# TimZaman/dotaclient

Hardware: NVIDIA H100
Metric: optimizer_steps_per_sec (higher is better)
Workload: dtype f32

## Files before the change

dotaclient_b200/_lib.py:

```python
import ctypes
import os

_HERE = os.path.dirname(os.path.abspath(__file__))
LIB_PATH = os.path.join(_HERE, "libdotaclient_b200.so")

_c = ctypes
_vp, _i32, _i64, _f32, _f64, _sz = _c.c_void_p, _c.c_int, _c.c_int64, _c.c_float, _c.c_double, _c.c_size_t
_ptr5 = _c.c_void_p * 5


class GatherDesc(_c.Structure):
    _fields_ = [("src", _vp), ("dst", _vp), ("outer", _i64), ("src_cols", _i64), ("row_bytes", _i64)]

SIGNATURES = {
    "dc_version": (_i32, []),
    "dc_last_error": (_c.c_char_p, []),
    "dc_device_info": (_i32, [_c.POINTER(_i32)] * 3),
    "dc_gae_scan": (_i32, [_vp, _i32, _vp, _vp, _i32, _vp, _vp, _f64, _f64, _vp, _vp, _vp]),
    "dc_vtrace_scan": (_i32, [_vp, _i32, _vp, _vp, _vp, _vp, _i32, _vp, _vp, _f64, _f64, _f64, _f64, _vp, _vp, _vp, _vp]),
    "dc_gae_scan_indexed": (_i32, [_vp, _i32, _vp, _i64, _vp, _vp, _i32, _vp, _vp, _f64, _f64, _vp, _vp, _vp]),
    "dc_vtrace_scan_indexed": (_i32, [_vp, _i32, _vp, _i64, _vp, _vp, _vp, _vp, _i32, _vp, _vp, _f64, _f64, _f64, _f64, _vp,
                                      _vp, _vp, _vp]),
    "dc_upgo_scan": (_i32, [_vp, _i32, _vp, _vp, _vp, _vp, _i32, _vp, _vp, _f64, _f64, _f64, _vp, _vp, _vp]),
    "dc_upgo_scan_indexed": (_i32, [_vp, _i32, _vp, _i64, _vp, _vp, _vp, _vp, _i32, _vp, _vp, _f64, _f64, _f64, _vp, _vp,
                                    _vp]),
    "dc_gae_scan_heads": (_i32, [_vp, _i32, _vp, _i32, _vp, _vp, _i32, _vp, _vp, _vp, _f64, _vp, _vp, _vp]),
    "dc_gae_scan_heads_indexed": (_i32, [_vp, _i32, _vp, _i32, _vp, _i64, _vp, _vp, _i32, _vp, _vp, _vp, _f64, _vp, _vp,
                                         _vp]),
    "dc_value_heads_loss": (_i32, [_vp, _i64, _vp, _vp, _vp, _i64, _i32, _vp, _vp, _i64, _vp, _vp, _vp, _vp, _vp]),
    "dc_gather_columns": (_i32, [_c.POINTER(GatherDesc), _i32, _vp, _i64, _vp]),
    "dc_gather_columns_fill": (_i32, [_c.POINTER(GatherDesc), _i32, _vp, _i64, _vp]),
    "dc_refresh_states": (_i32, [_i32, _i32, _vp, _vp, _i64, _i64, _vp, _vp, _vp, _i64, _i64, _i64, _vp, _vp, _vp, _vp, _vp,
                                 _vp, _vp]),
    "dc_rnn_workspace_bytes": (_sz, [_i32, _i32, _i32]),
    "dc_rnn_seq_fwd": (_i32, [_i32, _vp, _vp, _vp, _vp, _vp, _i32, _i32, _i32, _vp, _vp]),
    "dc_rnn_seq_bwd": (_i32, [_i32, _vp, _vp, _vp, _vp, _vp, _vp, _vp, _vp, _vp, _i32, _i32, _i32, _vp, _vp]),
    "dc_rnn_seq_fwd_reset": (_i32, [_i32, _vp, _vp, _vp, _vp, _vp, _vp, _vp, _vp, _i32, _i32, _i32, _i32, _vp, _vp]),
    "dc_rnn_seq_bwd_reset": (_i32, [_i32, _vp, _vp, _vp, _vp, _vp, _vp, _vp, _vp, _vp, _vp, _vp, _i32, _i32, _i32, _i32, _vp,
                                    _vp]),
    "dc_gemm_tf32x3_supported": (_i32, [_i64, _i32, _i32]),
    "dc_gemm_tf32x3": (_i32, [_vp, _i32, _vp, _i32, _vp, _vp, _i32, _i64, _i32, _i32, _i32, _vp]),
    "dc_gemm_wgrad_workspace_bytes": (_sz, [_i32, _i32]),
    "dc_gemm_wgrad_tf32x3": (_i32, [_vp, _i32, _vp, _i32, _i64, _i32, _i32, _vp, _i32, _vp, _i32, _vp, _vp]),
    "dc_gemm_tf32x3_rows": (_i32, [_vp, _i32, _vp, _i32, _vp, _vp, _vp, _i32, _i64, _vp, _vp, _i32, _i32, _i32, _i32, _vp]),
    "dc_gemm_wgrad_tf32x3_rows": (_i32, [_vp, _i32, _vp, _i32, _vp, _i64, _vp, _i32, _i32, _vp, _i32, _vp, _i32, _vp, _vp]),
    "dc_unit_basic_bwd_workspace_bytes": (_sz, []),
    "dc_env_fwd": (_i32, [_vp, _vp, _vp, _vp, _i32, _i64, _vp]),
    "dc_env_bwd_workspace_bytes": (_sz, []),
    "dc_env_bwd": (_i32, [_vp, _vp, _i32, _vp, _vp, _vp, _i64, _vp, _vp]),
    "dc_unit_wgrad_routed": (_i32, [_vp, _vp, _i32, _vp, _vp, _i64, _i32, _vp, _vp, _vp, _vp]),
    "dc_unit_dgrad_fused": (_i32, [_vp, _vp, _i32, _vp, _vp, _i32, _vp, _vp, _vp, _vp, _vp, _i64, _i32, _vp, _vp, _i32, _vp, _vp]),
    "dc_unit_dgrad_fused_mask": (_i32, [_vp, _vp, _i32, _vp, _vp, _i32, _vp, _vp, _vp, _vp, _vp, _vp, _i64, _i32, _vp, _vp, _i32, _vp,
                                        _vp]),
    "dc_gemm_unit_max": (_i32, [_vp, _vp, _vp, _vp, _vp, _i32, _vp, _i64, _i32, _vp]),
    "dc_unit_embed_fwd": (_i32, [_vp, _vp, _vp, _vp, _vp, _vp, _vp, _vp, _i32, _vp, _i64, _i32, _vp]),
    "dc_unit_embed_fwd_mask": (_i32, [_vp, _vp, _vp, _vp, _vp, _vp, _vp, _vp, _vp, _i32, _vp, _i64, _i32, _vp]),
    "dc_target_unit_q_fwd": (_i32, [_vp, _i32, _c.c_void_p * 6, _vp, _vp, _vp, _i64, _vp]),
    "dc_target_unit_q_bwd": (_i32, [_vp, _c.c_void_p * 6, _vp, _vp, _vp, _i32, _i64, _vp]),
    "dc_target_unit_q_fwd_rows": (_i32, [_vp, _i32, _c.c_void_p * 6, _vp, _vp, _vp, _i64, _vp, _vp, _vp]),
    "dc_target_unit_q_bwd_rows": (_i32, [_vp, _c.c_void_p * 6, _vp, _vp, _vp, _i32, _i64, _vp, _vp, _vp]),
    "dc_target_rows_workspace_bytes": (_sz, [_i64]),
    "dc_target_rows": (_i32, [_vp, _vp, _i64, _vp, _vp, _vp, _vp, _vp]),
    "dc_rows_zero_inactive": (_i32, [_vp, _i64, _vp, _i32, _i32, _vp]),
    "dc_ppo_loss_fwd_bwd": (_i32, [_ptr5, _ptr5, _ptr5, _vp, _vp, _vp, _vp, _i64, _f32, _f32, _f32, _ptr5, _vp, _vp,
                                   _vp, _vp, _vp]),
    "dc_ppo_loss_fwd_bwd_strided": (_i32, [_ptr5, _c.c_int64 * 5, _ptr5, _ptr5, _vp, _vp, _vp, _vp, _i64, _i64, _f32, _f32, _f32,
                                           _ptr5, _c.c_int64 * 5, _vp, _i64, _vp, _vp, _vp, _vp]),
    "dc_ppo_loss_fwd_bwd_dev": (_i32, [_ptr5, _c.c_int64 * 5, _ptr5, _ptr5, _vp, _vp, _vp, _vp, _i64, _vp, _i64, _vp,
                                       _ptr5, _c.c_int64 * 5, _vp, _i64, _vp, _vp, _vp, _vp, _vp]),
    "dc_ppo_loss_fwd_bwd_masked": (_i32, [_ptr5, _c.c_int64 * 5, _ptr5, _ptr5, _vp, _vp, _vp, _vp, _i64, _vp, _vp, _i64,
                                          _vp, _ptr5, _c.c_int64 * 5, _vp, _i64, _vp, _vp, _vp, _vp, _vp]),
    "dc_ppo_loss_fwd_bwd_joint": (_i32, [_ptr5, _c.c_int64 * 5, _ptr5, _ptr5, _vp, _vp, _vp, _vp, _i64, _vp, _vp, _i64,
                                         _vp, _ptr5, _c.c_int64 * 5, _vp, _i64, _vp, _vp, _vp, _vp, _vp]),
    "dc_ppo_loss_fwd_bwd_kl": (_i32, [_ptr5, _c.c_int64 * 5, _ptr5, _ptr5, _vp, _vp, _vp, _vp, _vp, _i64, _vp, _vp, _i64,
                                      _vp, _i32, _ptr5, _c.c_int64 * 5, _vp, _i64, _vp, _vp, _vp, _vp, _vp, _vp]),
    "dc_ppo_loss_fwd_bwd_teacher": (_i32, [_ptr5, _c.c_int64 * 5, _ptr5, _ptr5, _vp, _vp, _vp, _vp, _vp, _vp, _i64, _vp,
                                           _vp, _i64, _vp, _vp, _i32, _ptr5, _c.c_int64 * 5, _vp, _i64, _vp, _vp, _vp,
                                           _vp, _vp, _vp, _vp]),
    "dc_ppo_loss_fwd_bwd_dual_clip": (_i32, [_ptr5, _c.c_int64 * 5, _ptr5, _ptr5, _vp, _vp, _vp, _vp, _vp, _vp, _i64,
                                             _vp, _vp, _i64, _vp, _vp, _vp, _i32, _ptr5, _c.c_int64 * 5, _vp, _i64, _vp,
                                             _vp, _vp, _vp, _vp, _vp, _vp, _vp]),
    "dc_ppo_loss_fwd_bwd_bc": (_i32, [_ptr5, _c.c_int64 * 5, _ptr5, _ptr5, _vp, _vp, _vp, _i64, _vp, _vp, _i64, _vp, _ptr5,
                                      _c.c_int64 * 5, _vp, _i64, _vp, _vp, _vp, _vp, _vp, _vp]),
    "dc_selected_logp_rows": (_i32, [_ptr5, _ptr5, _ptr5, _i64, _vp, _vp, _vp]),
    "dc_value_norm_stats": (_i32, [_vp, _vp, _i64, _vp, _vp]),
    "dc_value_denorm": (_i32, [_vp, _i64, _i64, _f64, _f64, _vp, _vp]),
    "dc_value_head_rescale": (_i32, [_vp, _i64, _vp, _f64, _f64, _f64, _f64, _vp]),
    "dc_selected_logp": (_i32, [_ptr5, _ptr5, _ptr5, _i64, _vp, _vp]),
    "dc_select_actions": (_i32, [_ptr5, _c.c_int64 * 5, _ptr5, _vp, _i64, _vp, _vp, _vp]),
    "dc_grad_flags": (_i32, [_vp, _i64, _vp, _i32, _vp, _vp]),
    "dc_grad_finish": (_i32, [_vp, _vp, _vp, _vp, _vp, _vp, _vp, _vp, _i32, _i64, _f64, _f64, _f64, _f64, _f64, _vp, _vp,
                              _vp, _vp]),
    "dc_grad_finish_dev": (_i32, [_vp, _vp, _vp, _vp, _vp, _vp, _vp, _vp, _i32, _i64, _vp, _f64, _f64, _f64, _vp, _vp, _vp,
                                  _vp]),
    "dc_grad_finish_kl": (_i32, [_vp, _vp, _vp, _vp, _vp, _vp, _vp, _vp, _i32, _i64, _vp, _f64, _f64, _f64, _vp, _vp, _vp,
                                 _vp]),
}

PPO_WORKSPACE_BYTES = 512
FINISH_WORKSPACE_BYTES = 1024
LOSS_SLOTS = 16
HPARAM_SLOTS = 10
HP_LR, HP_E_CLIP, HP_ENTROPY_COEF, HP_VF_COEF, HP_MAX_GRAD_NORM, HP_VALUE_CLIP = range(6)
HP_VALUE_NORM_MEAN, HP_VALUE_NORM_STD = 6, 7
HP_KL_COEF, HP_KL_STOP = 8, 9
PPO_STATS_SLOTS = 24
STAT_APPROX_KL, STAT_CLIP_FRACTION, STAT_EXPLAINED_VAR = 0, 6, 12
STAT_JOINT_APPROX_KL, STAT_JOINT_CLIP_FRACTION = 13, 14
STAT_KL, STAT_KL_PENALTY = 16, 22
KL_ROW_FLOATS = 65
TEACHER_STATS_SLOTS = 7
BC_STATS_SLOTS = 12
DUAL_CLIP_STATS_SLOTS = 7
FINISH_KL_METRICS = 6
VTRACE_STATS_SLOTS = 8
UPGO_STATS_SLOTS = 3
VALUE_HEADS_MAX = 10
VALUE_HEADS_STATS_SLOTS = 20
VALUE_HEADS_WORKSPACE_BYTES = 131072
GATHER_MAX_TENSORS = 32
REFRESH_MAX_LAYERS = 16
MAX_PARAM_TENSORS = 96

_lib = None


class NativeLibraryError(RuntimeError):
    pass


def load():
    global _lib
    if _lib is not None:
        return _lib
    if not os.path.exists(LIB_PATH):
        raise NativeLibraryError(
            "%s not found: build it with `python -m dotaclient_b200.build` (needs nvcc, sm_90a). "
            "dotaclient_b200 has no CPU fallback." % LIB_PATH)
    lib = ctypes.CDLL(LIB_PATH)
    for name, (res, args) in SIGNATURES.items():
        try:
            fn = getattr(lib, name)
        except AttributeError:
            continue
        fn.restype = res
        fn.argtypes = args
    _lib = lib
    return lib


def exported(name):
    lib = load()
    return hasattr(lib, name)


def check(rc, what):
    if rc != 0:
        msg = load().dc_last_error()
        raise RuntimeError("%s failed (code %d): %s" % (what, rc, msg.decode() if msg else "?"))


def ptr(t):
    return None if t is None else t.data_ptr()


def ptr5(tensors):
    return _ptr5(*[t.data_ptr() if t is not None else None for t in tensors])


def stream_ptr():
    import torch
    return torch.cuda.current_stream().cuda_stream
```

dotaclient_b200/csrc/gemm_tf32x3.cu:

```cuda
#include "dc_common.cuh"
#include "unit_basic.cuh"

namespace {

constexpr int BM = 128, BN = 128, BK = 32;
constexpr int kStages = 2;
constexpr int kTileBytes = BM * BK * 4;
constexpr int kStageBytes = 4 * kTileBytes;
constexpr int kProducerThreads = 128;
constexpr int kProducerGroups = kStages;
constexpr int kConsumerWarp0 = 4 * kProducerGroups;
constexpr int kConsumerThreads = 256;
constexpr int kThreads = kConsumerWarp0 * 32 + kConsumerThreads;
constexpr int kLdS = BN + 8;
constexpr int kDIn = kUnitFeatures;
constexpr size_t kOffStaging = (size_t)kStages * kStageBytes;
constexpr size_t kOffBars = kOffStaging + (size_t)BM * kLdS * 4;
constexpr size_t kSmemBytes = kOffBars + 128 + 1024 ;

#define DC_ACC8(b) "+f"(d[b]), "+f"(d[b + 1]), "+f"(d[b + 2]), "+f"(d[b + 3]), "+f"(d[b + 4]), "+f"(d[b + 5]), "+f"(d[b + 6]), "+f"(d[b + 7])
__device__ __forceinline__ void wgmma_m64n128k8(float (&d)[64], uint64_t desc_a, uint64_t desc_b) {
    asm volatile(
        "{\n\t.reg .pred p;\n\tsetp.ne.b32 p, %66, 0;\n\t"
        "wgmma.mma_async.sync.aligned.m64n128k8.f32.tf32.tf32 "
        "{%0, %1, %2, %3, %4, %5, %6, %7, %8, %9, %10, %11, %12, %13, %14, %15, "
        "%16, %17, %18, %19, %20, %21, %22, %23, %24, %25, %26, %27, %28, %29, %30, %31, "
        "%32, %33, %34, %35, %36, %37, %38, %39, %40, %41, %42, %43, %44, %45, %46, %47, "
        "%48, %49, %50, %51, %52, %53, %54, %55, %56, %57, %58, %59, %60, %61, %62, %63}, "
        "%64, %65, p, 1, 1;\n\t}\n"
        : DC_ACC8(0), DC_ACC8(8), DC_ACC8(16), DC_ACC8(24), DC_ACC8(32), DC_ACC8(40), DC_ACC8(48), DC_ACC8(56)
        : "l"(desc_a), "l"(desc_b), "r"(1));
}
#undef DC_ACC8

__device__ __forceinline__ void mma_stage(float (&d)[64], uint32_t stage_base, int wg) {
    const uint64_t a_hi = dc_wgmma_desc(stage_base + wg * (64 * 128)), a_lo = dc_wgmma_desc(stage_base + kTileBytes + wg * (64 * 128));
    const uint64_t b_hi = dc_wgmma_desc(stage_base + 2 * kTileBytes), b_lo = dc_wgmma_desc(stage_base + 3 * kTileBytes);
#pragma unroll
    for (int i = 0; i < 64; ++i) dc_reg_fence(d[i]);
    dc_wgmma_fence();
#pragma unroll
    for (int ks = 0; ks < BK / 8; ++ks) {
        const uint64_t adv = (uint64_t)(ks * 2);
        wgmma_m64n128k8(d, a_lo + adv, b_hi + adv);
        wgmma_m64n128k8(d, a_hi + adv, b_lo + adv);
        wgmma_m64n128k8(d, a_hi + adv, b_hi + adv);
    }
    dc_wgmma_commit();
    dc_wgmma_wait0();
#pragma unroll
    for (int i = 0; i < 64; ++i) dc_reg_fence(d[i]);
}

__device__ __forceinline__ void consume(float (&d)[64], unsigned char *tiles, uint64_t *full, uint64_t *empty, uint32_t &c, int n,
                                       int wg, int lane) {
#pragma unroll
    for (int i = 0; i < 64; ++i) d[i] = 0.f;
    for (int kc = 0; kc < n; ++kc, ++c) {
        const int s = c % kStages;
        dc_mbar_wait(&full[s], (c / kStages) & 1);
        __syncwarp();
        mma_stage(d, dc_smem_u32(tiles + (size_t)s * kStageBytes), wg);
        __syncwarp();
        if (lane == 0) dc_mbar_arrive(&empty[s]);
    }
}

__device__ __forceinline__ void consumer_sync() { asm volatile("bar.sync 1, %0;" ::"n"(kConsumerThreads) : "memory"); }

__device__ __forceinline__ void stage_acc(const float (&d)[64], float *S, int ct) {
    const int wg = ct >> 7, w = (ct >> 5) & 3, lane = ct & 31;
    const int r0 = 64 * wg + 16 * w + (lane >> 2), c0 = 2 * (lane & 3);
#pragma unroll
    for (int i = 0; i < 64; i += 2) {
        const int row = r0 + 8 * ((i >> 1) & 1), col = 8 * (i >> 2) + c0;
        *reinterpret_cast<float2 *>(S + row * kLdS + col) = make_float2(d[i], d[i + 1]);
    }
}

__device__ __forceinline__ void init_ring(uint64_t *bars) {
    if (threadIdx.x == 0) {
        for (int s = 0; s < kStages; ++s) { dc_mbar_init(&bars[s], 4); dc_mbar_init(&bars[kStages + s], kConsumerThreads / 32); }
        asm volatile("fence.mbarrier_init.release.cluster;" ::: "memory");
    }
    __syncthreads();
}
__device__ __forceinline__ unsigned char *smem_base(unsigned char *raw) {
    return reinterpret_cast<unsigned char *>((reinterpret_cast<uintptr_t>(raw) + 1023) & ~(uintptr_t)1023);
}
template <typename F>
__device__ __forceinline__ void produce(uint64_t *full, uint64_t *empty, uint32_t c, int lane, F &&store) {
    const int s = c % kStages;
    dc_mbar_wait(&empty[s], ((c / kStages) & 1) ^ 1);
    store(s);
    asm volatile("fence.proxy.async.shared::cta;" ::: "memory");
    __syncwarp();
    if (lane == 0) dc_mbar_arrive(&full[s]);
}

__device__ __forceinline__ void tile_load_k(const float *__restrict__ src, int ld, int row0, int rows_total, int k0, int t,
                                            float4 (&v)[8], const int *__restrict__ rows = nullptr) {
    const int c = t & 7, r0 = t >> 3;
#pragma unroll
    for (int i = 0; i < 8; ++i) {
        const int r = r0 + 16 * i;
        const bool ok = row0 + r < rows_total;
        const size_t sr = rows != nullptr && ok ? (size_t)__ldg(rows + row0 + r) : (size_t)(row0 + r);
        v[i] = ok ? __ldg(reinterpret_cast<const float4 *>(src + sr * ld + k0) + c) : make_float4(0.f, 0.f, 0.f, 0.f);
    }
}
__device__ __forceinline__ void tile_store_k(const float4 (&v)[8], unsigned char *dst_hi, unsigned char *dst_lo, int t) {
    const int c = t & 7, r0 = t >> 3;
#pragma unroll
    for (int i = 0; i < 8; ++i) {
        const int r = r0 + 16 * i;
        const int off = r * 128 + ((c ^ (r & 7)) << 4);
        float4 hi, lo;
        hi.x = dc_tf32_rna(v[i].x); hi.y = dc_tf32_rna(v[i].y); hi.z = dc_tf32_rna(v[i].z); hi.w = dc_tf32_rna(v[i].w);
        lo.x = v[i].x - hi.x; lo.y = v[i].y - hi.y; lo.z = v[i].z - hi.z; lo.w = v[i].w - hi.w;
        *reinterpret_cast<float4 *>(dst_hi + off) = hi;
        *reinterpret_cast<float4 *>(dst_lo + off) = lo;
    }
}

template <int NU>
struct DembRaw {
    static constexpr int kP = NU == 16 ? 1 : 2;
    static constexpr int kU = NU == 16 ? 8 : NU;
    float4 d[kP], d2[kP], a[kP];
    uint32_t am[kP];
    float g[kP][kU];
    bool ok[kP];
};
template <>
struct DembRaw<1> {
    float4 v[8];
};

template <int NU>
__device__ __forceinline__ void demb_fetch(DembRaw<NU> &raw, const float *__restrict__ dx, const float *__restrict__ dx2, int ld_dx,
                                           const uint8_t *__restrict__ argmax, const float *__restrict__ dl, int ld_dl,
                                           const float *__restrict__ att, int tok0, int n_tok, int k0, int t) {
    const float4 zero4 = make_float4(0.f, 0.f, 0.f, 0.f);
    if constexpr (NU == 1) {
        const int c = t & 7, r0 = t >> 3;
#pragma unroll
        for (int i = 0; i < 8; ++i) {
            const int n = tok0 + r0 + 16 * i;
            const bool ok = n < n_tok;
            const size_t nn = (size_t)min(n, n_tok - 1);
            float4 d = dx != nullptr ? __ldg(reinterpret_cast<const float4 *>(dx + nn * ld_dx + k0) + c) : zero4;
            if (dx2 != nullptr) {
                const float4 d2 = __ldg(reinterpret_cast<const float4 *>(dx2 + nn * ld_dx + k0) + c);
                d.x += d2.x; d.y += d2.y; d.z += d2.z; d.w += d2.w;
            }
            const float4 a4 = dl != nullptr ? __ldg(reinterpret_cast<const float4 *>(att + nn * 128 + k0) + c) : zero4;
            const float gl = dl != nullptr ? __ldg(dl + nn * ld_dl) : 0.f;
            raw.v[i] = ok ? make_float4(fmaf(gl, a4.x, d.x), fmaf(gl, a4.y, d.y), fmaf(gl, a4.z, d.z), fmaf(gl, a4.w, d.w)) : zero4;
        }
    } else {
        constexpr int kTileToks = (BM - BM % NU) / NU;
#pragma unroll
        for (int k = 0; k < DembRaw<NU>::kP; ++k) {
            const int p = t + kProducerThreads * k;
            const int c = p & 7, tokl = NU == 16 ? p >> 4 : p >> 3;
            const int u0 = NU == 16 ? ((p >> 3) & 1) * 8 : 0;
            const bool active = tokl < kTileToks;
            const int n = tok0 + tokl;
            raw.ok[k] = active && n < n_tok;
            const size_t nn = (size_t)min(n, n_tok - 1);
            float4 d = (active && dx != nullptr) ? __ldg(reinterpret_cast<const float4 *>(dx + nn * ld_dx + k0) + c) : zero4;
            const float4 d2 = (active && dx2 != nullptr) ? __ldg(reinterpret_cast<const float4 *>(dx2 + nn * ld_dx + k0) + c) : zero4;
            if constexpr (NU == 16) {
                raw.d2[k] = d2;
            } else {
                d.x += d2.x; d.y += d2.y; d.z += d2.z; d.w += d2.w;
            }
            raw.d[k] = d;
            raw.am[k] = (active && dx != nullptr) ? __ldg(reinterpret_cast<const uint32_t *>(argmax + nn * 128 + k0) + c) : 0u;
            raw.a[k] = (active && dl != nullptr) ? __ldg(reinterpret_cast<const float4 *>(att + nn * 128 + k0) + c) : zero4;
#pragma unroll
            for (int j = 0; j < DembRaw<NU>::kU; ++j) raw.g[k][j] = (active && dl != nullptr) ? __ldg(dl + nn * ld_dl + u0 + j) : 0.f;
        }
    }
}

__device__ __forceinline__ void store_hi_lo(unsigned char *dst_hi, unsigned char *dst_lo, int off, float4 o) {
    float4 hi, lo;
    hi.x = dc_tf32_rna(o.x); hi.y = dc_tf32_rna(o.y); hi.z = dc_tf32_rna(o.z); hi.w = dc_tf32_rna(o.w);
    lo.x = o.x - hi.x; lo.y = o.y - hi.y; lo.z = o.z - hi.z; lo.w = o.w - hi.w;
    *reinterpret_cast<float4 *>(dst_hi + off) = hi;
    *reinterpret_cast<float4 *>(dst_lo + off) = lo;
}

template <int NU>
__device__ __forceinline__ void demb_store(const DembRaw<NU> &raw, unsigned char *dst_hi, unsigned char *dst_lo, int t) {
    if constexpr (NU == 1) {
        tile_store_k(raw.v, dst_hi, dst_lo, t);
    } else {
        constexpr int kTileRows = BM - BM % NU, kTileToks = kTileRows / NU;
        const float4 zero4 = make_float4(0.f, 0.f, 0.f, 0.f);
#pragma unroll
        for (int k = 0; k < DembRaw<NU>::kP; ++k) {
            const int p = t + kProducerThreads * k;
            const int c = p & 7, tokl = NU == 16 ? p >> 4 : p >> 3;
            const int u0 = NU == 16 ? ((p >> 3) & 1) * 8 : 0;
            if (tokl < kTileToks) {
                float4 d = raw.d[k];
                if constexpr (NU == 16) { d.x += raw.d2[k].x; d.y += raw.d2[k].y; d.z += raw.d2[k].z; d.w += raw.d2[k].w; }
                const float4 a = raw.a[k];
                const uint32_t am = raw.am[k];
#pragma unroll
                for (int j = 0; j < DembRaw<NU>::kU; ++j) {
                    const int u = u0 + j, r = tokl * NU + u;
                    const float gl = raw.g[k][j];
                    float4 o;
                    o.x = fmaf(gl, a.x, (int)(am & 0xffu) == u ? d.x : 0.f);
                    o.y = fmaf(gl, a.y, (int)((am >> 8) & 0xffu) == u ? d.y : 0.f);
                    o.z = fmaf(gl, a.z, (int)((am >> 16) & 0xffu) == u ? d.z : 0.f);
                    o.w = fmaf(gl, a.w, (int)(am >> 24) == u ? d.w : 0.f);
                    store_hi_lo(dst_hi, dst_lo, r * 128 + ((c ^ (r & 7)) << 4), raw.ok[k] ? o : zero4);
                }
            }
        }
        if constexpr (kTileRows < BM) {
            if (t < (BM - kTileRows) * 8) {
                const int r = kTileRows + (t >> 3), c = t & 7;
                store_hi_lo(dst_hi, dst_lo, r * 128 + ((c ^ (r & 7)) << 4), zero4);
            }
        }
    }
}

__device__ __forceinline__ void store_row_k(const float (&v)[32], unsigned char *dst_hi, unsigned char *dst_lo, int row) {
#pragma unroll
    for (int c = 0; c < 8; ++c) {
        const int off = row * 128 + ((c ^ (row & 7)) << 4);
        float4 hi, lo;
        hi.x = dc_tf32_rna(v[4 * c]); hi.y = dc_tf32_rna(v[4 * c + 1]); hi.z = dc_tf32_rna(v[4 * c + 2]); hi.w = dc_tf32_rna(v[4 * c + 3]);
        lo.x = v[4 * c] - hi.x; lo.y = v[4 * c + 1] - hi.y; lo.z = v[4 * c + 2] - hi.z; lo.w = v[4 * c + 3] - hi.w;
        *reinterpret_cast<float4 *>(dst_hi + off) = hi;
        *reinterpret_cast<float4 *>(dst_lo + off) = lo;
    }
}

template <bool kDevM = false>
__global__ void __launch_bounds__(kThreads, 1) gemm_tf32x3_kernel(const float *__restrict__ A, int lda,
                                                                  const float *__restrict__ B, int ldb,
                                                                  const float *__restrict__ bias, float *__restrict__ C,
                                                                  int ldc, int M, int N, int K, int relu, int ksplit,
                                                                  long long c_split_stride, const int *__restrict__ m_dev = nullptr,
                                                                  const int *__restrict__ a_rows = nullptr, const int *__restrict__ rows = nullptr,
                                                                  float *__restrict__ C_rows = nullptr) {
    constexpr int kTileRows = BM;
    if constexpr (kDevM) M = min(M, __ldg(m_dev));
    extern __shared__ unsigned char smem_raw[];
    unsigned char *tiles = smem_base(smem_raw);
    float *S = reinterpret_cast<float *>(tiles + kOffStaging);
    uint64_t *full = reinterpret_cast<uint64_t *>(tiles + kOffBars), *empty = full + kStages;

    const int warp = threadIdx.x >> 5, lane = threadIdx.x & 31;
    const int m_blocks = (M + kTileRows - 1) / kTileRows, n_blocks = (N + BN - 1) / BN, k_chunks = K / BK / ksplit;
    const int tiles_mn = m_blocks * n_blocks, tiles_total = tiles_mn * ksplit;
    init_ring(full);

    if (warp < kConsumerWarp0) {
        const int t = threadIdx.x & (kProducerThreads - 1), g = warp >> 2;
        uint32_t c = 0;
        for (int tile = blockIdx.x; tile < tiles_total; tile += gridDim.x) {
            const int tmn = tile % tiles_mn, kc0 = (tile / tiles_mn) * k_chunks;
            const int m0 = (tmn / n_blocks) * kTileRows, n0 = (tmn % n_blocks) * BN;
            for (int kc = 0; kc < k_chunks; ++kc, ++c) {
                if ((int)(c % kProducerGroups) != g) continue;
                float4 va[8], vb[8];
                tile_load_k(A, lda, m0, M, (kc0 + kc) * BK, t, va, kDevM ? a_rows : nullptr);
                tile_load_k(B, ldb, n0, N, (kc0 + kc) * BK, t, vb);
                produce(full, empty, c, lane, [&](int s) {
                    unsigned char *st = tiles + (size_t)s * kStageBytes;
                    tile_store_k(va, st, st + kTileBytes, t);
                    tile_store_k(vb, st + 2 * kTileBytes, st + 3 * kTileBytes, t);
                });
            }
        }
    } else {
        const int ct = threadIdx.x - kConsumerWarp0 * 32, wg = ct >> 7, cw = ct >> 5;
        float d[64];
        uint32_t c = 0;
        for (int tile = blockIdx.x; tile < tiles_total; tile += gridDim.x) {
            const int tmn = tile % tiles_mn, sp = tile / tiles_mn;
            const int m0 = (tmn / n_blocks) * kTileRows, n0 = (tmn % n_blocks) * BN;
            consume(d, tiles, full, empty, c, k_chunks, wg, lane);
            consumer_sync();
            stage_acc(d, S, ct);
            consumer_sync();
            const bool lane_in = n0 + 4 * lane < N;
            const bool has_bias = bias != nullptr && sp == 0 && lane_in;
            const float4 b4 = has_bias ? __ldg(reinterpret_cast<const float4 *>(bias + n0) + lane) : make_float4(0.f, 0.f, 0.f, 0.f);
            float *cbase = C + (size_t)sp * (size_t)c_split_stride + n0 + 4 * lane;
            for (int r = cw; lane_in && r < BM && m0 + r < M; r += kConsumerThreads / 32) {
                float4 v = *reinterpret_cast<const float4 *>(S + r * kLdS + 4 * lane);
                if (has_bias) { v.x += b4.x; v.y += b4.y; v.z += b4.z; v.w += b4.w; }
                if (relu) { v.x = fmaxf(v.x, 0.f); v.y = fmaxf(v.y, 0.f); v.z = fmaxf(v.z, 0.f); v.w = fmaxf(v.w, 0.f); }
                if (!kDevM || C != nullptr) *reinterpret_cast<float4 *>(cbase + (size_t)(m0 + r) * ldc) = v;
                if (kDevM && C_rows != nullptr)
                    *reinterpret_cast<float4 *>(C_rows + (size_t)__ldg(rows + m0 + r) * ldc + n0 + 4 * lane) = v;
            }
        }
    }
}

constexpr int kWsRows = 64;
constexpr int kWsStages = 8;
constexpr int kWsChunkBytes = kWsRows * BK * 4;
constexpr int kWsThreads = kConsumerThreads + 128;
constexpr int kWsLdS = 40;
constexpr size_t kWsOffRing = (size_t)4 * 2 * kTileBytes;
constexpr size_t kWsOffStaging = kWsOffRing + (size_t)kWsStages * kWsChunkBytes;
constexpr size_t kWsOffBars = kWsOffStaging + (size_t)(kConsumerThreads / 32) * 16 * kWsLdS * 4;
constexpr size_t kWsSmemBytes = kWsOffBars + 2 * kWsStages * 8 + 1024 ;
constexpr size_t kWsOffUnits = kWsOffBars + 2 * kWsStages * 8;
constexpr size_t kWsGenSmemBytes = kWsOffUnits + (size_t)4 * kWsRows * kDIn * 4 + 1024 ;
static_assert(kWsSmemBytes <= 227 * 1024 && kWsGenSmemBytes <= 227 * 1024, "weight-stationary GEMM exceeds the shared-memory opt-in");
static_assert(kWsOffUnits % 16 == 0, "unit rows are staged with 16-byte stores");

struct GenA {
    const float *units, *w_b, *b_b;
    float *basic_out;
    uint32_t *mask_out;
};

__device__ __forceinline__ void cp_async16(uint32_t dst, const void *src, uint32_t src_bytes) {
    asm volatile("cp.async.cg.shared.global [%0], [%1], 16, %2;" ::"r"(dst), "l"(src), "r"(src_bytes) : "memory");
}
__device__ __forceinline__ void cp_async_arrive(uint64_t *bar) {
    asm volatile("cp.async.mbarrier.arrive.noinc.shared::cta.b64 [%0];" ::"r"(dc_smem_u32(bar)) : "memory");
}

#define DC_ACC8(b) "+f"(d[b]), "+f"(d[b + 1]), "+f"(d[b + 2]), "+f"(d[b + 3]), "+f"(d[b + 4]), "+f"(d[b + 5]), "+f"(d[b + 6]), "+f"(d[b + 7])
__device__ __forceinline__ void wgmma_m64n128k8_rs(float (&d)[64], uint32_t a0, uint32_t a1, uint32_t a2, uint32_t a3, uint64_t desc_b) {
    asm volatile(
        "{\n\t.reg .pred p;\n\tsetp.ne.b32 p, %69, 0;\n\t"
        "wgmma.mma_async.sync.aligned.m64n128k8.f32.tf32.tf32 "
        "{%0, %1, %2, %3, %4, %5, %6, %7, %8, %9, %10, %11, %12, %13, %14, %15, "
        "%16, %17, %18, %19, %20, %21, %22, %23, %24, %25, %26, %27, %28, %29, %30, %31, "
        "%32, %33, %34, %35, %36, %37, %38, %39, %40, %41, %42, %43, %44, %45, %46, %47, "
        "%48, %49, %50, %51, %52, %53, %54, %55, %56, %57, %58, %59, %60, %61, %62, %63}, "
        "{%64, %65, %66, %67}, %68, p, 1, 1;\n\t}\n"
        : DC_ACC8(0), DC_ACC8(8), DC_ACC8(16), DC_ACC8(24), DC_ACC8(32), DC_ACC8(40), DC_ACC8(48), DC_ACC8(56)
        : "r"(a0), "r"(a1), "r"(a2), "r"(a3), "l"(desc_b), "r"(1));
}
#undef DC_ACC8

__device__ __forceinline__ void ws_fetch(float (&v)[16], const float *chunk, int rlo, int rhi, bool hi_ok, int q) {
#pragma unroll
    for (int ks = 0; ks < BK / 8; ++ks) {
#pragma unroll
        for (int h = 0; h < 2; ++h) {
            const int j = 2 * ks + h;
            v[4 * ks + 2 * h] = chunk[rlo * BK + ((j ^ (rlo & 7)) << 2) + q];
            v[4 * ks + 2 * h + 1] = hi_ok ? chunk[rhi * BK + ((j ^ (rhi & 7)) << 2) + q] : 0.f;
        }
    }
}

template <int NU, bool kGenA, bool kDevM = false>
__global__ void __launch_bounds__(kWsThreads, 1) gemm_ws_kernel(const float *__restrict__ A, int lda,
                                                                const float *__restrict__ B, int ldb,
                                                                const float *__restrict__ bias, float *__restrict__ C,
                                                                int ldc, int M, int N, int K, int relu,
                                                                float *__restrict__ C_copy, uint8_t *__restrict__ argmax, GenA gen,
                                                                const int *__restrict__ m_dev = nullptr, const int *__restrict__ a_rows = nullptr,
                                                                const int *__restrict__ rows = nullptr, float *__restrict__ C_rows = nullptr) {
    if constexpr (kDevM) M = min(M, __ldg(m_dev));
    constexpr int kWarpRows = NU == 5 ? 15 : 16;
    constexpr int kTileRows = 4 * kWarpRows;
    extern __shared__ unsigned char smem_raw[];
    unsigned char *sm = smem_base(smem_raw);
    unsigned char *ring = sm + kWsOffRing;
    uint64_t *full = reinterpret_cast<uint64_t *>(sm + kWsOffBars), *empty = full + kWsStages;

    const int warp = threadIdx.x >> 5, lane = threadIdx.x & 31;
    const int n_blocks = (N + BN - 1) / BN, m_blocks = (M + kTileRows - 1) / kTileRows, k_chunks = K / BK;
    const int n0 = (blockIdx.x % n_blocks) * BN, mb0 = blockIdx.x / n_blocks, mstride = gridDim.x / n_blocks;
    if (threadIdx.x == 0) {
        for (int s = 0; s < kWsStages; ++s) { dc_mbar_init(&full[s], kGenA ? 1 : 128); dc_mbar_init(&empty[s], 4); }
        asm volatile("fence.mbarrier_init.release.cluster;" ::: "memory");
    }
    __syncthreads();

    if constexpr (kGenA) if (warp >= kConsumerThreads / 32) {
        const int kc = warp - kConsumerThreads / 32, ch = lane & 7, r0 = lane >> 3;
        const int j0 = kc * BK + 4 * ch;
        float wb[4][kDIn], bb[4];
#pragma unroll
        for (int e = 0; e < 4; ++e) {
            bb[e] = __ldg(gen.b_b + j0 + e);
#pragma unroll
            for (int k = 0; k < kDIn; ++k) wb[e][k] = __ldg(gen.w_b + (j0 + e) * kDIn + k);
        }
        float4 *su = reinterpret_cast<float4 *>(sm + kWsOffUnits) + kc * (kWsRows * kDIn / 4);
        const float4 *units4 = reinterpret_cast<const float4 *>(gen.units);
        constexpr int kU4 = kWsRows * kDIn / 4 / 32;
        float4 nxt[kU4];
        auto fetch = [&](int mb) {
            const bool live = mb < m_blocks;
            const int m0 = live ? mb * kTileRows : 0;
#pragma unroll
            for (int i = 0; i < kU4; ++i) {
                const int idx = lane + 32 * i, r = idx / 3;
                nxt[i] = (live && r < kTileRows && m0 + r < M) ? __ldg(units4 + (size_t)m0 * 3 + idx) : make_float4(0.f, 0.f, 0.f, 0.f);
            }
        };
        fetch(mb0);
        uint32_t c = kc;
        for (int mb = mb0; mb < m_blocks; mb += mstride, c += 4) {
            const int m0 = mb * kTileRows;
            __syncwarp();
#pragma unroll
            for (int i = 0; i < kU4; ++i) su[lane + 32 * i] = nxt[i];
            __syncwarp();
            fetch(mb + mstride);
            const int s = c % kWsStages;
            dc_mbar_wait(&empty[s], ((c / kWsStages) & 1) ^ 1);
            unsigned char *chunk = ring + (size_t)s * kWsChunkBytes;
#pragma unroll 4
            for (int i = 0; i < kWsRows / 4; ++i) {
                const int r = r0 + 4 * i;
                const bool ok = r < kTileRows && m0 + r < M;
                const float4 u0 = su[3 * r], u1 = su[3 * r + 1], u2 = su[3 * r + 2];
                const float u[kDIn] = {u0.x, u0.y, u0.z, u0.w, u1.x, u1.y, u1.z, u1.w, u2.x, u2.y, u2.z, u2.w};
                float4 v = make_float4(dc_unit_basic(u, wb[0], bb[0]), dc_unit_basic(u, wb[1], bb[1]), dc_unit_basic(u, wb[2], bb[2]),
                                       dc_unit_basic(u, wb[3], bb[3]));
                if (!ok) v = make_float4(0.f, 0.f, 0.f, 0.f);
                *reinterpret_cast<float4 *>(chunk + r * 128 + ((ch ^ (r & 7)) << 4)) = v;
                if (gen.basic_out != nullptr && ok) *reinterpret_cast<float4 *>(gen.basic_out + (size_t)(m0 + r) * BN + j0) = v;
            }
            __syncwarp();
            if (lane == 0) dc_mbar_arrive(&full[s]);
        }
        return;
    }
    if constexpr (!kGenA) if (warp >= kConsumerThreads / 32) {
        const int p = threadIdx.x - kConsumerThreads, ch = p & 7;
        uint32_t c = 0;
        for (int mb = mb0; mb < m_blocks; mb += mstride) {
            const int m0 = mb * kTileRows;
            for (int kc = 0; kc < k_chunks; ++kc, ++c) {
                const int s = c % kWsStages;
                dc_mbar_wait(&empty[s], ((c / kWsStages) & 1) ^ 1);
                const uint32_t dst = dc_smem_u32(ring + (size_t)s * kWsChunkBytes);
#pragma unroll
                for (int i = 0; i < kWsRows / 16; ++i) {
                    const int r = (p >> 3) + 16 * i;
                    const bool ok = r < kTileRows && m0 + r < M;
                    const size_t ar = kDevM && a_rows != nullptr && ok ? (size_t)__ldg(a_rows + m0 + r) : (size_t)(m0 + r);
                    const float *src = A + (ok ? ar * lda : 0) + kc * BK + 4 * ch;
                    cp_async16(dst + r * 128 + ((ch ^ (r & 7)) << 4), src, ok ? 16u : 0u);
                }
                cp_async_arrive(&full[s]);
            }
        }
        asm volatile("cp.async.wait_all;" ::: "memory");
        return;
    }

    const int wg = warp >> 2, w4 = warp & 3, t = threadIdx.x & 127, q = lane & 3, g8 = lane >> 2;
    {
        for (int kc = wg; kc < k_chunks; kc += 2) {
            float4 vb[8];
            tile_load_k(B, ldb, n0, N, kc * BK, t, vb);
            tile_store_k(vb, sm + (size_t)kc * 2 * kTileBytes, sm + (size_t)kc * 2 * kTileBytes + kTileBytes, t);
        }
        asm volatile("fence.proxy.async.shared::cta;" ::: "memory");
        consumer_sync();
    }
    const uint32_t w_base = dc_smem_u32(sm);
    const int rlo = kWarpRows * w4 + g8, rhi = rlo + 8;
    const bool hi_ok = NU != 5 || g8 < 7;
    float *Sw = reinterpret_cast<float *>(sm + kWsOffStaging) + warp * 16 * kWsLdS;
    float d[64];
    uint32_t c = 0;
    int i = 0;
    for (int mb = mb0; mb < m_blocks; mb += mstride, ++i, c += k_chunks) {
        if ((i & 1) != wg) continue;
        const int m0 = mb * kTileRows;
        uint32_t mask_lo = 0, mask_hi = 0;
#pragma unroll
        for (int j = 0; j < 64; ++j) d[j] = 0.f;
        float v[16];
        uint32_t ahi[16], alo[16];
        {
            const int s = c % kWsStages;
            dc_mbar_wait(&full[s], (c / kWsStages) & 1);
            ws_fetch(v, reinterpret_cast<const float *>(ring + (size_t)s * kWsChunkBytes), rlo, rhi, hi_ok, q);
        }
        for (int kc = 0; kc < k_chunks; ++kc) {
#pragma unroll
            for (int j = 0; j < 16; ++j) {
                const float h = dc_tf32_rna(v[j]);
                ahi[j] = __float_as_uint(h);
                alo[j] = __float_as_uint(v[j] - h);
            }
            __syncwarp();
            if (lane == 0) dc_mbar_arrive(&empty[(c + kc) % kWsStages]);
#pragma unroll
            for (int j = 0; j < 64; ++j) dc_reg_fence(d[j]);
            dc_wgmma_fence();
            const uint64_t b_hi = dc_wgmma_desc(w_base + kc * 2 * kTileBytes), b_lo = dc_wgmma_desc(w_base + kc * 2 * kTileBytes + kTileBytes);
#pragma unroll
            for (int ks = 0; ks < BK / 8; ++ks) {
                const uint64_t adv = (uint64_t)(ks * 2);
                wgmma_m64n128k8_rs(d, alo[4 * ks], alo[4 * ks + 1], alo[4 * ks + 2], alo[4 * ks + 3], b_hi + adv);
                wgmma_m64n128k8_rs(d, ahi[4 * ks], ahi[4 * ks + 1], ahi[4 * ks + 2], ahi[4 * ks + 3], b_lo + adv);
                wgmma_m64n128k8_rs(d, ahi[4 * ks], ahi[4 * ks + 1], ahi[4 * ks + 2], ahi[4 * ks + 3], b_hi + adv);
            }
            dc_wgmma_commit();
            if (kGenA && gen.mask_out != nullptr) {
                uint32_t lo = 0, hi = 0;
#pragma unroll
                for (int ks = 0; ks < BK / 8; ++ks) {
#pragma unroll
                    for (int h = 0; h < 2; ++h) {
                        lo |= v[4 * ks + 2 * h] > 0.f ? 1u << (2 * ks + h) : 0u;
                        hi |= v[4 * ks + 2 * h + 1] > 0.f ? 1u << (2 * ks + h) : 0u;
                    }
                }
                mask_lo |= lo << (8 * kc);
                mask_hi |= hi << (8 * kc);
            }
            if (kc + 1 < k_chunks) {
                const uint32_t cn = c + kc + 1;
                const int s = cn % kWsStages;
                dc_mbar_wait(&full[s], (cn / kWsStages) & 1);
                ws_fetch(v, reinterpret_cast<const float *>(ring + (size_t)s * kWsChunkBytes), rlo, rhi, hi_ok, q);
            }
            dc_wgmma_wait0();
#pragma unroll
            for (int j = 0; j < 16; ++j) asm volatile("" : "+r"(ahi[j]), "+r"(alo[j])::"memory");
#pragma unroll
            for (int j = 0; j < 64; ++j) dc_reg_fence(d[j]);
        }
        if (kGenA && gen.mask_out != nullptr) {
            if (m0 + rlo < M) gen.mask_out[(size_t)(m0 + rlo) * 4 + q] = mask_lo;
            if (hi_ok && m0 + rhi < M) gen.mask_out[(size_t)(m0 + rhi) * 4 + q] = mask_hi;
        }

        if constexpr (NU == 0) {
            const int row_lo = m0 + rlo, row_hi = m0 + rhi;
            float *c_lo = row_lo < M ? C + (size_t)row_lo * ldc : nullptr, *c_hi = row_hi < M ? C + (size_t)row_hi * ldc : nullptr;
            float *r_lo = nullptr, *r_hi = nullptr;
            if constexpr (kDevM) {
                if (C == nullptr) c_lo = c_hi = nullptr;
                if (C_rows != nullptr) {
                    if (row_lo < M) r_lo = C_rows + (size_t)__ldg(rows + row_lo) * ldc;
                    if (row_hi < M) r_hi = C_rows + (size_t)__ldg(rows + row_hi) * ldc;
                }
            }
#pragma unroll
            for (int g = 0; g < BN / 8; ++g) {
                const int col = n0 + 8 * g + 2 * q;
                if (col >= N) break;
                const float2 b2 = bias != nullptr ? __ldg(reinterpret_cast<const float2 *>(bias + col)) : make_float2(0.f, 0.f);
                float2 lo = make_float2(d[4 * g], d[4 * g + 1]), hi = make_float2(d[4 * g + 2], d[4 * g + 3]);
                if (bias != nullptr) { lo.x += b2.x; lo.y += b2.y; hi.x += b2.x; hi.y += b2.y; }
                if (relu) { lo.x = fmaxf(lo.x, 0.f); lo.y = fmaxf(lo.y, 0.f); hi.x = fmaxf(hi.x, 0.f); hi.y = fmaxf(hi.y, 0.f); }
                if (c_lo) *reinterpret_cast<float2 *>(c_lo + col) = lo;
                if (c_hi) *reinterpret_cast<float2 *>(c_hi + col) = hi;
                if (kDevM && r_lo) *reinterpret_cast<float2 *>(r_lo + col) = lo;
                if (kDevM && r_hi) *reinterpret_cast<float2 *>(r_hi + col) = hi;
            }
        } else {
            constexpr int kToks = kWarpRows / NU;
            const int tok0 = m0 / NU + kToks * w4, n_tok = M / NU;
#pragma unroll
            for (int b = 0; b < BN / 32; ++b) {
#pragma unroll
                for (int g = 0; g < 4; ++g) {
                    const int j = 4 * (4 * b + g);
                    *reinterpret_cast<float2 *>(Sw + g8 * kWsLdS + 8 * g + 2 * q) = make_float2(d[j], d[j + 1]);
                    *reinterpret_cast<float2 *>(Sw + (g8 + 8) * kWsLdS + 8 * g + 2 * q) = make_float2(d[j + 2], d[j + 3]);
                }
                __syncwarp();
                const int col = 32 * b + lane;
                const float bias_f = __ldg(bias + col);
#pragma unroll
                for (int tk = 0; tk < kToks; ++tk) {
                    const int tok = tok0 + tk;
                    if (tok >= n_tok) break;
                    const float *p = Sw + tk * NU * kWsLdS + lane;
                    float best = p[0];
                    int best_u = 0;
#pragma unroll
                    for (int u = 1; u < NU; ++u) {
                        const float x = p[u * kWsLdS];
                        if (x > best) { best = x; best_u = u; }
                    }
                    const float o = best + bias_f;
                    C[(size_t)tok * ldc + col] = o;
                    if (C_copy) C_copy[(size_t)tok * ldc + col] = o;
                    argmax[(size_t)tok * BN + col] = (uint8_t)best_u;
                }
                __syncwarp();
            }
        }
    }
}

constexpr int kDgN = 16;
constexpr int kDgUTile = kDgN * BK * 4;
constexpr int kDgStageBytes = 2 * kTileBytes;
constexpr size_t kDgOffRing = (size_t)(BN / BK) * 2 * kTileBytes;
constexpr size_t kDgOffU = kDgOffRing + (size_t)kStages * kDgStageBytes;
constexpr int kDgFlush = 32;
constexpr int kDgMaskLd = BM + 8;
constexpr size_t kDgOffMask = kDgOffU + (size_t)2 * (BM / BK) * kDgUTile;
constexpr size_t kDgOffWb = kDgOffMask + (size_t)4 * kDgMaskLd * 4;
constexpr size_t kDgOffBars = kDgOffWb + (size_t)BN * (kDIn + 1) * 4;
constexpr size_t kDgSmemBytes = kDgOffBars + 2 * (kStages + 1) * 8 + 1024 ;
static_assert(kDgSmemBytes <= 227 * 1024, "unit data-gradient kernel exceeds the shared-memory opt-in");
static_assert(kDgOffU % 1024 == 0 && kDgUTile % 1024 == 0, "the swizzled U tiles need 1024-byte alignment");

__device__ __forceinline__ void wgmma_wait1() { asm volatile("wgmma.wait_group.sync.aligned 1;" ::: "memory"); }

__device__ __forceinline__ void wgmma_m64n16k8_rs(float (&d)[8], const uint32_t (&a)[4], uint64_t desc_b) {
    asm volatile(
        "{\n\t.reg .pred p;\n\tsetp.ne.b32 p, %13, 0;\n\t"
        "wgmma.mma_async.sync.aligned.m64n16k8.f32.tf32.tf32 {%0, %1, %2, %3, %4, %5, %6, %7}, {%8, %9, %10, %11}, %12, p, 1, 1;\n\t}\n"
        : "+f"(d[0]), "+f"(d[1]), "+f"(d[2]), "+f"(d[3]), "+f"(d[4]), "+f"(d[5]), "+f"(d[6]), "+f"(d[7])
        : "r"(a[0]), "r"(a[1]), "r"(a[2]), "r"(a[3]), "l"(desc_b), "r"(1));
}

struct DgAux {
    float4 u[3];
    uint32_t m[4];
    bool ok;
};

template <bool kMask>
__device__ __forceinline__ void aux_fetch(DgAux &x, const float *__restrict__ units, const uint32_t *__restrict__ mask, int m0,
                                          int rows_valid, int t) {
    const float4 zero4 = make_float4(0.f, 0.f, 0.f, 0.f);
    x.ok = t < rows_valid;
    const size_t row = (size_t)(m0 + (x.ok ? t : 0));
#pragma unroll
    for (int i = 0; i < 3; ++i) x.u[i] = x.ok ? __ldg(reinterpret_cast<const float4 *>(units) + row * 3 + i) : zero4;
    if constexpr (kMask) {
        const uint4 w = x.ok ? __ldg(reinterpret_cast<const uint4 *>(mask) + row) : make_uint4(0u, 0u, 0u, 0u);
        x.m[0] = w.x; x.m[1] = w.y; x.m[2] = w.z; x.m[3] = w.w;
    }
}

__device__ __forceinline__ void aux_recompute_mask(DgAux &x, const float *sw, const float *sb) {
    const float u[kDIn] = {x.u[0].x, x.u[0].y, x.u[0].z, x.u[0].w, x.u[1].x, x.u[1].y, x.u[1].z, x.u[1].w, x.u[2].x, x.u[2].y, x.u[2].z, x.u[2].w};
#pragma unroll
    for (int w = 0; w < 4; ++w) {
        uint32_t bits = 0;
#pragma unroll 4
        for (int i = 0; i < 32; ++i) {
            const int j = 4 * i + w;
            const float4 *wr4 = reinterpret_cast<const float4 *>(sw + j * kDIn);
            const float4 w0 = wr4[0], w1 = wr4[1], w2 = wr4[2];
            const float wr[kDIn] = {w0.x, w0.y, w0.z, w0.w, w1.x, w1.y, w1.z, w1.w, w2.x, w2.y, w2.z, w2.w};
            bits |= (dc_unit_basic(u, wr, sb[j]) > 0.f ? 1u : 0u) << i;
        }
        x.m[w] = x.ok ? bits : 0u;
    }
}

__device__ __forceinline__ void aux_store(const DgAux &x, unsigned char *sm_u, uint32_t *sm_mask, int t) {
    const int k = 8 * (t >> 3) + ((t & 7) >> 1) + 4 * (t & 1), kk = k & 31;
    unsigned char *base = sm_u + (k >> 5) * kDgUTile + (kk & 3) * 4;
    const float v[kDgN] = {x.u[0].x, x.u[0].y, x.u[0].z, x.u[0].w, x.u[1].x, x.u[1].y, x.u[1].z, x.u[1].w,
                           x.u[2].x, x.u[2].y, x.u[2].z, x.u[2].w, x.ok ? 1.f : 0.f, 0.f, 0.f, 0.f};
#pragma unroll
    for (int n = 0; n < kDgN; ++n) {
        const float hi = dc_tf32_rna(v[n]);
        const int off = n * 128 + (((kk >> 2) ^ (n & 7)) << 4);
        *reinterpret_cast<float *>(base + off) = hi;
        *reinterpret_cast<float *>(base + (BM / BK) * kDgUTile + off) = v[n] - hi;
    }
#pragma unroll
    for (int w = 0; w < 4; ++w) sm_mask[w * kDgMaskLd + t] = x.m[w];
}

template <int NU, bool kMask>
__global__ void __launch_bounds__(kThreads, 1) unit_dgrad_kernel(const float *__restrict__ dx, const float *__restrict__ dx2, int ld_dx,
                                                                 const uint8_t *__restrict__ argmax,
                                                                 const float *__restrict__ dl, int ld_dl,
                                                                 const float *__restrict__ att,
                                                                 const float *__restrict__ Wt, const float *__restrict__ units,
                                                                 const uint32_t *__restrict__ mask,
                                                                 const float *__restrict__ w_b, const float *__restrict__ b_b,
                                                                 int n_tok, float *__restrict__ partial) {
    constexpr int kTileRows = BM - BM % NU, kTileToks = kTileRows / NU;
    constexpr int k_chunks = BN / BK;
    extern __shared__ unsigned char smem_raw[];
    unsigned char *sm = smem_base(smem_raw);
    unsigned char *ring = sm + kDgOffRing, *sm_u = sm + kDgOffU;
    uint32_t *sm_mask = reinterpret_cast<uint32_t *>(sm + kDgOffMask);
    float *sm_wb = reinterpret_cast<float *>(sm + kDgOffWb), *sm_bb = sm_wb + BN * kDIn;
    uint64_t *full = reinterpret_cast<uint64_t *>(sm + kDgOffBars), *empty = full + kStages;
    uint64_t *ufull = empty + kStages, *uempty = ufull + 1;

    const int warp = threadIdx.x >> 5, lane = threadIdx.x & 31;
    const int M = n_tok * NU;
    const int m_blocks = (M + kTileRows - 1) / kTileRows;
    if constexpr (!kMask) {
        for (int i = threadIdx.x; i < BN * kDIn; i += kThreads) sm_wb[i] = __ldg(w_b + i);
        for (int i = threadIdx.x; i < BN; i += kThreads) sm_bb[i] = __ldg(b_b + i);
    }
    if (threadIdx.x == 0) {
        dc_mbar_init(ufull, 4);
        dc_mbar_init(uempty, kConsumerThreads / 32);
    }
    init_ring(full);

    if (warp < kConsumerWarp0) {
        const int t = threadIdx.x & (kProducerThreads - 1), g = warp >> 2;
        uint32_t c = 0;
        int it = 0;
        for (int mb = blockIdx.x; mb < m_blocks; mb += gridDim.x, ++it) {
            const int tok0 = mb * kTileToks, m0 = mb * kTileRows;
            for (int kc = 0; kc < k_chunks; ++kc, ++c) {
                if ((int)(c % kProducerGroups) != g) continue;
                DembRaw<NU> raw;
                DgAux aux;
                demb_fetch<NU>(raw, dx, dx2, ld_dx, argmax, dl, ld_dl, att, tok0, n_tok, kc * BK, t);
                if (kc == 0) aux_fetch<kMask>(aux, units, mask, m0, min(kTileRows, M - m0), t);
                produce(full, empty, c, lane, [&](int s) { demb_store<NU>(raw, ring + (size_t)s * kDgStageBytes, ring + (size_t)s * kDgStageBytes + kTileBytes, t); });
                if (kc == 0) {
                    if constexpr (!kMask) aux_recompute_mask(aux, sm_wb, sm_bb);
                    dc_mbar_wait(uempty, (it & 1) ^ 1);
                    aux_store(aux, sm_u, sm_mask, t);
                    asm volatile("fence.proxy.async.shared::cta;" ::: "memory");
                    __syncwarp();
                    if (lane == 0) dc_mbar_arrive(ufull);
                }
            }
        }
    } else {
        const int ct = threadIdx.x - kConsumerWarp0 * 32, wg = ct >> 7, w4 = (ct >> 5) & 3, t = ct & 127, q4 = lane & 3;
        for (int kc = wg; kc < k_chunks; kc += 2) {
            float4 vb[8];
            tile_load_k(Wt, BN, 0, BN, kc * BK, t, vb);
            tile_store_k(vb, sm + (size_t)kc * 2 * kTileBytes, sm + (size_t)kc * 2 * kTileBytes + kTileBytes, t);
        }
        asm volatile("fence.proxy.async.shared::cta;" ::: "memory");
        consumer_sync();
        const uint32_t w_base = dc_smem_u32(sm) + wg * (64 * 128), ring_base = dc_smem_u32(ring), u_base = dc_smem_u32(sm_u);
        const int j_lo = 64 * wg + 16 * w4 + (lane >> 2);
        const uint32_t bit_lo = 1u << (j_lo >> 2), bit_hi = bit_lo << 2;
        const uint32_t *mrow = sm_mask + (j_lo & 3) * kDgMaskLd + 2 * q4;
        float acc[8];
#pragma unroll
        for (int i = 0; i < 8; ++i) acc[i] = 0.f;
        float *pp = partial + (size_t)blockIdx.x * BN * (kDIn + 1);
        const auto flush = [&](bool add) {
#pragma unroll
            for (int i = 0; i < 8; ++i) {
                const int j = j_lo + 8 * ((i >> 1) & 1), n = 8 * (i >> 2) + 2 * q4 + (i & 1);
                if (n <= kDIn) {
                    if (add) atomicAdd(pp + j * (kDIn + 1) + n, acc[i]);
                    else pp[j * (kDIn + 1) + n] = acc[i];
                }
                acc[i] = 0.f;
            }
#pragma unroll
            for (int i = 0; i < 8; ++i) dc_reg_fence(acc[i]);
        };
        float d[64];
        uint32_t c = 0;
        int it = 0;
        for (int mb = blockIdx.x; mb < m_blocks; mb += gridDim.x, ++it) {
#pragma unroll
            for (int i = 0; i < 64; ++i) d[i] = 0.f;
#pragma unroll 1
            for (int kc = 0; kc < k_chunks; ++kc, ++c) {
                const int s = c % kStages;
                dc_mbar_wait(&full[s], (c / kStages) & 1);
#pragma unroll
                for (int i = 0; i < 64; ++i) dc_reg_fence(d[i]);
                dc_wgmma_fence();
                const uint64_t a_hi = dc_wgmma_desc(w_base + kc * 2 * kTileBytes), a_lo = dc_wgmma_desc(w_base + kc * 2 * kTileBytes + kTileBytes);
                const uint64_t b_hi = dc_wgmma_desc(ring_base + s * kDgStageBytes), b_lo = dc_wgmma_desc(ring_base + s * kDgStageBytes + kTileBytes);
#pragma unroll
                for (int ks = 0; ks < BK / 8; ++ks) {
                    const uint64_t adv = (uint64_t)(ks * 2);
                    wgmma_m64n128k8(d, a_hi + adv, b_lo + adv);
                    wgmma_m64n128k8(d, a_lo + adv, b_hi + adv);
                    wgmma_m64n128k8(d, a_hi + adv, b_hi + adv);
                }
                dc_wgmma_commit();
                if (kc > 0) {
                    wgmma_wait1();
                    __syncwarp();
                    if (lane == 0) dc_mbar_arrive(&empty[(c - 1) % kStages]);
                }
            }
            dc_wgmma_wait0();
#pragma unroll
            for (int i = 0; i < 64; ++i) dc_reg_fence(d[i]);
            __syncwarp();
            if (lane == 0) dc_mbar_arrive(&empty[(c - 1) % kStages]);

            dc_mbar_wait(ufull, it & 1);
            uint32_t ghi[2][4], glo[2][4];
#pragma unroll
            for (int q = 0; q < BM / 8; ++q) {
                const int b = q & 1;
                const uint2 mw = *reinterpret_cast<const uint2 *>(mrow + 8 * q);
                const float gv[4] = {(mw.x & bit_lo) ? d[4 * q] : 0.f, (mw.x & bit_hi) ? d[4 * q + 2] : 0.f,
                                     (mw.y & bit_lo) ? d[4 * q + 1] : 0.f, (mw.y & bit_hi) ? d[4 * q + 3] : 0.f};
#pragma unroll
                for (int e = 0; e < 4; ++e) {
                    const float h = dc_tf32_rna(gv[e]);
                    ghi[b][e] = __float_as_uint(h);
                    glo[b][e] = __float_as_uint(gv[e] - h);
                }
                dc_wgmma_fence();
                const uint64_t u_hi = dc_wgmma_desc(u_base + (q >> 2) * kDgUTile) + 2 * (q & 3);
                const uint64_t u_lo = dc_wgmma_desc(u_base + (BM / BK + (q >> 2)) * kDgUTile) + 2 * (q & 3);
                wgmma_m64n16k8_rs(acc, glo[b], u_hi);
                wgmma_m64n16k8_rs(acc, ghi[b], u_lo);
                wgmma_m64n16k8_rs(acc, ghi[b], u_hi);
                dc_wgmma_commit();
                wgmma_wait1();
#pragma unroll
                for (int e = 0; e < 4; ++e) asm volatile("" : "+r"(ghi[b ^ 1][e]), "+r"(glo[b ^ 1][e])::"memory");
            }
            dc_wgmma_wait0();
#pragma unroll
            for (int i = 0; i < 8; ++i) dc_reg_fence(acc[i]);
            __syncwarp();
            if (lane == 0) dc_mbar_arrive(uempty);
            if ((it + 1) % kDgFlush == 0 && mb + (int)gridDim.x < m_blocks) flush(it + 1 > kDgFlush);
        }
        flush(it > kDgFlush);
    }
}

constexpr int kWgStages = 4;
constexpr int kWgFlush = 128;
constexpr int kWgLdX = BN + 8;
constexpr int kWgStageBytes = 2 * kTileBytes + BK * kWgLdX * 4;
constexpr size_t kWgOffColsum = (size_t)kWgStages * kWgStageBytes;
constexpr size_t kWgOffBars = kWgOffColsum + 2 * BM * 4;
constexpr size_t kWgSmemBytes = kWgOffBars + 2 * kWgStages * 8 + 1024 ;
static_assert(kWgStageBytes % 1024 == 0, "the swizzled dY^T tiles need 1024-byte aligned slots");
static_assert(kWgSmemBytes <= 227 * 1024, "weight-gradient GEMM exceeds the shared-memory opt-in");

__device__ __forceinline__ float lds_f32(uint32_t addr) {
    float v;
    asm volatile("ld.shared.f32 %0, [%1];" : "=f"(v) : "r"(addr) : "memory");
    return v;
}

template <int NU, bool kDevT = false>
__global__ void __launch_bounds__(kThreads, 1) gemm_wgrad_kernel(const float *__restrict__ dY, int ldy,
                                                                 const float *__restrict__ dY2,
                                                                 const uint8_t *__restrict__ argmax,
                                                                 const float *__restrict__ X, int ldx, int T, int No,
                                                                 int Ni, int nsplit, float *__restrict__ part_w,
                                                                 float *__restrict__ part_b, const int *__restrict__ t_dev = nullptr,
                                                                 const int *__restrict__ x_rows = nullptr) {
    if constexpr (kDevT) T = min(T, __ldg(t_dev));
    constexpr int kTPC = NU > 0 ? BK / NU : 0;
    constexpr int kRPC = NU > 0 ? kTPC * NU : BK;
    extern __shared__ unsigned char smem_raw[];
    unsigned char *ring = smem_base(smem_raw);
    float *colsum_s = reinterpret_cast<float *>(ring + kWgOffColsum);
    uint64_t *full = reinterpret_cast<uint64_t *>(ring + kWgOffBars), *empty = full + kWgStages;

    const int warp = threadIdx.x >> 5, lane = threadIdx.x & 31;
    const int n_blocks = (Ni + BN - 1) / BN, tiles_mn = ((No + BM - 1) / BM) * n_blocks;
    const int tile = blockIdx.x % tiles_mn, split = blockIdx.x / tiles_mn;
    const int m0 = (tile / n_blocks) * BM, n0 = (tile % n_blocks) * BN;
    const int chunks_total = (T + kRPC - 1) / kRPC;
    const int my_chunks = split < chunks_total ? (chunks_total - split + nsplit - 1) / nsplit : 0;
    if (threadIdx.x == 0) {
        for (int s = 0; s < kWgStages; ++s) { dc_mbar_init(&full[s], kProducerThreads + 4); dc_mbar_init(&empty[s], kConsumerThreads / 32); }
        asm volatile("fence.mbarrier_init.release.cluster;" ::: "memory");
    }
    __syncthreads();

    if (warp < kConsumerWarp0) {
        const int g = warp >> 2, t = threadIdx.x & (kProducerThreads - 1), o = m0 + t;
        const bool o_in = o < No;
        const int xc = t & 31;
        const bool xc_in = n0 + 4 * xc < Ni;
        float cs = 0.f, cc = 0.f;
        for (int j = g; j < my_chunks; j += kProducerGroups) {
            float va[32];
            if constexpr (NU > 0) {
                const int tok0 = (split + j * nsplit) * kTPC, n_tok = T / NU;
                float dv[kTPC];
                int am[kTPC];
#pragma unroll
                for (int k = 0; k < kTPC; ++k) {
                    const bool ok = tok0 + k < n_tok;
                    const size_t at = (size_t)(tok0 + k) * ldy + o;
                    dv[k] = ok ? __ldg(dY + at) : 0.f;
                    if (ok && dY2 != nullptr) dv[k] += __ldg(dY2 + at);
                    am[k] = ok ? (int)__ldg(argmax + (size_t)(tok0 + k) * 128 + o) : 255;
                }
#pragma unroll
                for (int i = 0; i < 32; ++i) va[i] = (i < kRPC && am[i / NU] == i % NU) ? dv[i / NU] : 0.f;
            } else {
                const int t0 = (split + j * nsplit) * BK;
                const float *p = dY + (size_t)t0 * ldy + o;
#pragma unroll
                for (int i = 0; i < 32; ++i) va[i] = (o_in && t0 + i < T) ? __ldg(p + (size_t)i * ldy) : 0.f;
            }
            float sc = 0.f;
#pragma unroll
            for (int i = 0; i < 32; ++i) sc += va[i];
            const float y = sc - cc, cs_new = cs + y;
            cc = (cs_new - cs) - y;
            cs = cs_new;
            const int t0 = (split + j * nsplit) * kRPC, tend = min(T, t0 + kRPC);
            const int s = j % kWgStages;
            dc_mbar_wait(&empty[s], ((j / kWgStages) & 1) ^ 1);
            unsigned char *st = ring + (size_t)s * kWgStageBytes;
            const uint32_t xs = dc_smem_u32(st + 2 * kTileBytes);
#pragma unroll
            for (int r = 0; r < BK / 4; ++r) {
                const int row = (t >> 5) + 4 * r;
                const bool ok = xc_in && t0 + row < tend;
                const size_t xr = kDevT && x_rows != nullptr && ok ? (size_t)__ldg(x_rows + t0 + row) : (size_t)(t0 + row);
                cp_async16(xs + (row * kWgLdX + 4 * xc) * 4, X + (ok ? xr * ldx + n0 + 4 * xc : 0), ok ? 16u : 0u);
            }
            cp_async_arrive(&full[s]);
            store_row_k(va, st, st + kTileBytes, t);
            asm volatile("fence.proxy.async.shared::cta;" ::: "memory");
            __syncwarp();
            if (lane == 0) dc_mbar_arrive(&full[s]);
        }
        colsum_s[g * 128 + t] = cs;
        asm volatile("cp.async.wait_all;" ::: "memory");
    } else {
        const int ct = threadIdx.x - kConsumerWarp0 * 32, wg = ct >> 7, w4 = (ct >> 5) & 3, q = lane & 3;
        const int rlo = 64 * wg + 16 * w4 + (lane >> 2);
        float d[64];
#pragma unroll
        for (int i = 0; i < 64; ++i) d[i] = 0.f;
        uint32_t ahi[2][4] = {}, alo[2][4] = {};
#pragma unroll
        for (int i = 0; i < 64; ++i) dc_reg_fence(d[i]);
        float *pt = part_w + ((size_t)split * tiles_mn + tile) * BM * BN + ct * 4;
        const auto flush = [&](bool add) {
            dc_wgmma_wait0();
#pragma unroll
            for (int k = 0; k < 64; ++k) dc_reg_fence(d[k]);
            if (add) {
#pragma unroll
                for (int m = 0; m < 16; ++m)
                    asm volatile("red.global.add.v4.f32 [%0], {%1, %2, %3, %4};" ::"l"(pt + m * kConsumerThreads * 4), "f"(d[4 * m]),
                                 "f"(d[4 * m + 1]), "f"(d[4 * m + 2]), "f"(d[4 * m + 3]) : "memory");
            } else {
#pragma unroll
                for (int m = 0; m < 16; ++m)
                    *reinterpret_cast<float4 *>(pt + m * kConsumerThreads * 4) = make_float4(d[4 * m], d[4 * m + 1], d[4 * m + 2], d[4 * m + 3]);
            }
#pragma unroll
            for (int k = 0; k < 64; ++k) d[k] = 0.f;
#pragma unroll
            for (int k = 0; k < 64; ++k) dc_reg_fence(d[k]);
        };
        int j = 0;
        do {
            const int j_end = min(my_chunks, j + kWgFlush);
            for (; j < j_end; ++j) {
                const int s = j % kWgStages;
                dc_mbar_wait(&full[s], (j / kWgStages) & 1);
                const uint32_t st = dc_smem_u32(ring + (size_t)s * kWgStageBytes);
                const uint32_t xk = st + 2 * kTileBytes + (q * kWgLdX + rlo) * 4;
                float v[16];
#pragma unroll
                for (int ks = 0; ks < BK / 8; ++ks) {
                    const uint32_t x8 = xk + 8 * ks * kWgLdX * 4;
                    v[4 * ks] = lds_f32(x8);
                    v[4 * ks + 1] = lds_f32(x8 + 8 * 4);
                    v[4 * ks + 2] = lds_f32(x8 + 4 * kWgLdX * 4);
                    v[4 * ks + 3] = lds_f32(x8 + (4 * kWgLdX + 8) * 4);
                }
                const uint64_t b_hi = dc_wgmma_desc(st), b_lo = dc_wgmma_desc(st + kTileBytes);
#pragma unroll
                for (int ks = 0; ks < BK / 8; ++ks) {
                    const int b = ks & 1;
#pragma unroll
                    for (int e = 0; e < 4; ++e) {
                        const float h = dc_tf32_rna(v[4 * ks + e]);
                        ahi[b][e] = __float_as_uint(h);
                        alo[b][e] = __float_as_uint(v[4 * ks + e] - h);
                    }
                    dc_wgmma_fence();
                    const uint64_t adv = (uint64_t)(ks * 2);
                    wgmma_m64n128k8_rs(d, ahi[b][0], ahi[b][1], ahi[b][2], ahi[b][3], b_lo + adv);
                    wgmma_m64n128k8_rs(d, alo[b][0], alo[b][1], alo[b][2], alo[b][3], b_hi + adv);
                    wgmma_m64n128k8_rs(d, ahi[b][0], ahi[b][1], ahi[b][2], ahi[b][3], b_hi + adv);
                    dc_wgmma_commit();
                    wgmma_wait1();
#pragma unroll
                    for (int e = 0; e < 4; ++e) asm volatile("" : "+r"(ahi[b ^ 1][e]), "+r"(alo[b ^ 1][e])::"memory");
                    if (ks == 0 && j > 0) {
                        __syncwarp();
                        if (lane == 0) dc_mbar_arrive(&empty[(j - 1) % kWgStages]);
                    }
                }
            }
            flush(j > kWgFlush);
        } while (j < my_chunks);
    }
    __syncthreads();
    if (part_b != nullptr && n0 == 0 && threadIdx.x < 128 && m0 + (int)threadIdx.x < No)
        part_b[(size_t)split * No + m0 + threadIdx.x] = colsum_s[threadIdx.x] + colsum_s[128 + threadIdx.x];
}

constexpr int kRedRows = 8;
__global__ void __launch_bounds__(32 * kRedRows) wgrad_reduce_kernel(const float *__restrict__ part_w, const float *__restrict__ part_b,
                                                                     int nsplit, int No, int Ni, float *__restrict__ dW, int ldw,
                                                                     float *__restrict__ db, int accumulate) {
    __shared__ float4 sh[kRedRows][32];
    const int x = threadIdx.x & 31, y = threadIdx.x >> 5;
    const int n_blocks = (Ni + BN - 1) / BN, tiles_mn = ((No + BM - 1) / BM) * n_blocks;
    const int total4 = tiles_mn * (BM * BN / 4), bias4 = db != nullptr ? No / 4 : 0;
    const int idx = blockIdx.x * 32 + x;
    const float *src = nullptr;
    size_t stride = 0;
    if (idx < total4) {
        src = part_w + (size_t)idx * 4;
        stride = (size_t)tiles_mn * BM * BN;
    } else if (idx < total4 + bias4) {
        src = part_b + (size_t)(idx - total4) * 4;
        stride = (size_t)No;
    }
    float4 acc = make_float4(0.f, 0.f, 0.f, 0.f);
    if (src != nullptr) {
#pragma unroll 4
        for (int s = y; s < nsplit; s += kRedRows) {
            const float4 v = __ldg(reinterpret_cast<const float4 *>(src + (size_t)s * stride));
            acc.x += v.x; acc.y += v.y; acc.z += v.z; acc.w += v.w;
        }
    }
    sh[y][x] = acc;
    __syncthreads();
    if (y == 0 && src != nullptr) {
        if (idx < total4) {
            const int tile = idx / (BM * BN / 4), r = idx % (BM * BN / 4), m = r / kConsumerThreads, ct = r % kConsumerThreads;
            const int o = (tile / n_blocks) * BM + 8 * m + 2 * (ct & 3);
            const int i = (tile % n_blocks) * BN + 64 * (ct >> 7) + 16 * ((ct >> 5) & 3) + ((ct & 31) >> 2);
            float *p[4];
            float v[4];
#pragma unroll
            for (int e = 0; e < 4; ++e) {
                const int oe = o + (e & 1), ie = i + 8 * (e >> 1);
                p[e] = oe < No && ie < Ni ? dW + (size_t)oe * ldw + ie : nullptr;
                v[e] = accumulate && p[e] != nullptr ? *p[e] : 0.f;
            }
#pragma unroll
            for (int r = 0; r < kRedRows; ++r) { v[0] += sh[r][x].x; v[1] += sh[r][x].y; v[2] += sh[r][x].z; v[3] += sh[r][x].w; }
#pragma unroll
            for (int e = 0; e < 4; ++e)
                if (p[e] != nullptr) *p[e] = v[e];
        } else {
            float *dst = db + (size_t)(idx - total4) * 4;
            float4 t = accumulate ? *reinterpret_cast<const float4 *>(dst) : make_float4(0.f, 0.f, 0.f, 0.f);
#pragma unroll
            for (int r = 0; r < kRedRows; ++r) { t.x += sh[r][x].x; t.y += sh[r][x].y; t.z += sh[r][x].z; t.w += sh[r][x].w; }
            *reinterpret_cast<float4 *>(dst) = t;
        }
    }
}

}

extern "C" int dc_gemm_tf32x3_supported(int64_t M, int N, int K) { return M > 0 && N > 0 && K > 0 && N % 32 == 0 && K % BK == 0; }

struct RowList {
    const int *count, *a_rows, *rows;
    float *C_rows;
};

template <int NU, bool kGenA = false, bool kDevM = false>
static int launch_ws(const float *A, int lda, const float *B, int ldb, const float *bias, float *C, int ldc, int M, int N,
                     int K, int relu, float *C_copy, uint8_t *argmax, cudaStream_t st, GenA gen = GenA{}, RowList rl = RowList{}) {
    const int tile_rows = NU == 5 ? 60 : kWsRows;
    const int n_blocks = (N + BN - 1) / BN, m_blocks = (M + tile_rows - 1) / tile_rows;
    int per_block = dc_sm_count() / n_blocks;
    if (per_block < 1) per_block = 1;
    if (per_block > m_blocks) per_block = m_blocks;
    const size_t smem = kGenA ? kWsGenSmemBytes : kWsSmemBytes;
    DC_CUDA(cudaFuncSetAttribute(gemm_ws_kernel<NU, kGenA, kDevM>, cudaFuncAttributeMaxDynamicSharedMemorySize, (int)smem));
    gemm_ws_kernel<NU, kGenA, kDevM><<<n_blocks * per_block, kWsThreads, smem, st>>>(A, lda, B, ldb, bias, C, ldc, M, N, K, relu, C_copy,
                                                                                    argmax, gen, rl.count, rl.a_rows, rl.rows, rl.C_rows);
    DC_LAUNCH_OK();
    return DC_OK;
}

static int gemm_check_shape(const float *A, int lda, const float *B, int ldb, const float *bias, const float *C, int ldc, int64_t M,
                            int N, int K, const char *who) {
    DC_REQUIRE(dc_gemm_tf32x3_supported(M, N, K) && M < (1ll << 31) - BM, DC_EUNSUPPORTED,
               "%s: need N %% 32 == 0 and K %% 32 == 0 (M=%lld N=%d K=%d)", who, (long long)M, N, K);
    DC_REQUIRE(lda >= K && ldb >= K && ldc >= N && lda % 4 == 0 && ldb % 4 == 0 && ldc % 4 == 0, DC_EINVAL,
               "%s: leading dimensions must be >= extent and multiples of 4 floats", who);
    DC_REQUIRE(((uintptr_t)A & 15) == 0 && ((uintptr_t)B & 15) == 0 && ((uintptr_t)C & 15) == 0 && (!bias || ((uintptr_t)bias & 15) == 0),
               DC_EINVAL, "%s: pointers must be 16-byte aligned", who);
    return DC_OK;
}

static int gemm_check(const float *A, int lda, const float *B, int ldb, const float *bias, const float *C, int ldc, int64_t M, int N,
                      int K, const char *who) {
    DC_REQUIRE(A && B && C, DC_EINVAL, "%s: null pointer", who);
    return gemm_check_shape(A, lda, B, ldb, bias, C, ldc, M, N, K, who);
}

template <bool kDevM>
static int gemm_launch(const float *A, int lda, const float *B, int ldb, const float *bias, float *C, int ldc, int64_t M, int N, int K,
                       int relu, RowList rl, cudaStream_t st) {
    if (K <= 4 * BK) return launch_ws<0, false, kDevM>(A, lda, B, ldb, bias, C, ldc, (int)M, N, K, relu, nullptr, nullptr, st, GenA{}, rl);
    const int tiles = (int)((M + BM - 1) / BM) * ((N + BN - 1) / BN);
    DC_CUDA(cudaFuncSetAttribute(gemm_tf32x3_kernel<kDevM>, cudaFuncAttributeMaxDynamicSharedMemorySize, (int)kSmemBytes));
    const int grid = tiles < dc_sm_count() ? tiles : dc_sm_count();
    gemm_tf32x3_kernel<kDevM><<<grid, kThreads, kSmemBytes, st>>>(A, lda, B, ldb, bias, C, ldc, (int)M, N, K, relu, 1, 0, rl.count,
                                                                  rl.a_rows, rl.rows, rl.C_rows);
    DC_LAUNCH_OK();
    return DC_OK;
}

extern "C" int dc_gemm_tf32x3(const float *A, int lda, const float *B, int ldb, const float *bias, float *C, int ldc,
                              int64_t M, int N, int K, int relu, dc_stream_t stream) {
    const int rc = gemm_check(A, lda, B, ldb, bias, C, ldc, M, N, K, "dc_gemm_tf32x3");
    if (rc != DC_OK) return rc;
    return gemm_launch<false>(A, lda, B, ldb, bias, C, ldc, M, N, K, relu, RowList{}, dc_cu_stream(stream));
}

extern "C" int dc_gemm_tf32x3_rows(const float *A, int lda, const float *B, int ldb, const float *bias, float *C, float *C_rows, int ldc,
                                   int64_t M, const int32_t *count, const int32_t *rows, int gather_a, int N, int K, int relu,
                                   dc_stream_t stream) {
    DC_REQUIRE(A && B && count && (C || C_rows) && (rows || (!gather_a && !C_rows)), DC_EINVAL, "dc_gemm_tf32x3_rows: null pointer");
    DC_REQUIRE(((uintptr_t)C_rows & 15) == 0, DC_EINVAL, "dc_gemm_tf32x3_rows: pointers must be 16-byte aligned");
    const int rc = gemm_check_shape(A, lda, B, ldb, bias, C, ldc, M, N, K, "dc_gemm_tf32x3_rows");
    if (rc != DC_OK) return rc;
    return gemm_launch<true>(A, lda, B, ldb, bias, C, ldc, M, N, K, relu, RowList{count, gather_a ? rows : nullptr, rows, C_rows},
                             dc_cu_stream(stream));
}

int dc_gemm_tf32x3_splitk(const float *A, int lda, const float *B, int ldb, float *part, int64_t M, int N, int K, int ksplit,
                          bool first_call, cudaStream_t st) {
    DC_REQUIRE(A && B && part && ksplit >= 1 && N % BN == 0 && K % (BK * ksplit) == 0 && M > 0, DC_EINVAL,
               "dc_gemm_tf32x3_splitk: bad arguments (M=%lld N=%d K=%d ksplit=%d)", (long long)M, N, K, ksplit);
    if (first_call)
        DC_CUDA(cudaFuncSetAttribute(gemm_tf32x3_kernel<false>, cudaFuncAttributeMaxDynamicSharedMemorySize, (int)kSmemBytes));
    const int tiles = (int)((M + BM - 1) / BM) * (N / BN) * ksplit;
    const int grid = tiles < dc_sm_count() ? tiles : dc_sm_count();
    gemm_tf32x3_kernel<false><<<grid, kThreads, kSmemBytes, st>>>(A, lda, B, ldb, nullptr, part, N, (int)M, N, K, 0, ksplit, (long long)M * N);
    DC_LAUNCH_OK();
    return DC_OK;
}

static int wgrad_tiles(int No, int Ni) { return ((No + BM - 1) / BM) * ((Ni + BN - 1) / BN); }

static int wgrad_splits(int No, int Ni) {
    const int tiles_mn = wgrad_tiles(No, Ni);
    const int n = dc_sm_count() / tiles_mn;
    return n < 1 ? 1 : n;
}

extern "C" size_t dc_gemm_wgrad_workspace_bytes(int No, int Ni) {
    if (No <= 0 || Ni <= 0 || No % 32 || Ni % 32) return 0;
    const int nsplit = wgrad_splits(No, Ni);
    return ((size_t)nsplit * wgrad_tiles(No, Ni) * BM * BN + (size_t)nsplit * No) * sizeof(float);
}

template <bool kDevT>
static int wgrad_launch(const float *dY, int ldy, const float *X, int ldx, int64_t T, const int *t_dev, const int *x_rows, int No, int Ni,
                        float *dW, int ldw, float *db, int accumulate, void *workspace, dc_stream_t stream, const char *who) {
    DC_REQUIRE(dY && X && dW && workspace && (!kDevT || t_dev), DC_EINVAL, "%s: null pointer", who);
    DC_REQUIRE(T > 0 && T < (1ll << 31) - BK && No > 0 && Ni > 0 && No % 32 == 0 && Ni % 32 == 0, DC_EUNSUPPORTED,
               "%s: need No %% 32 == 0 and Ni %% 32 == 0 (T=%lld No=%d Ni=%d)", who, (long long)T, No, Ni);
    DC_REQUIRE(ldy >= No && ldx >= Ni && ldw >= Ni && ldy % 4 == 0 && ldx % 4 == 0 && ldw % 4 == 0, DC_EINVAL,
               "%s: bad leading dimension", who);
    DC_REQUIRE(((uintptr_t)dY & 15) == 0 && ((uintptr_t)X & 15) == 0 && ((uintptr_t)dW & 15) == 0 && ((uintptr_t)workspace & 15) == 0 &&
                   ((uintptr_t)db & 15) == 0,
               DC_EINVAL, "%s: pointers must be 16-byte aligned", who);
    const int tiles_mn = wgrad_tiles(No, Ni), nsplit = wgrad_splits(No, Ni);
    float *part_w = reinterpret_cast<float *>(workspace);
    float *part_b = db ? part_w + (size_t)nsplit * tiles_mn * BM * BN : nullptr;
    cudaStream_t st = dc_cu_stream(stream);
    DC_CUDA(cudaFuncSetAttribute(gemm_wgrad_kernel<0, kDevT>, cudaFuncAttributeMaxDynamicSharedMemorySize, (int)kWgSmemBytes));
    gemm_wgrad_kernel<0, kDevT><<<tiles_mn * nsplit, kThreads, kWgSmemBytes, st>>>(dY, ldy, nullptr, nullptr, X, ldx, (int)T, No, Ni,
                                                                                   nsplit, part_w, part_b, t_dev, x_rows);
    DC_LAUNCH_OK();
    const int total4 = tiles_mn * (BM * BN / 4) + (db ? No / 4 : 0);
    wgrad_reduce_kernel<<<(total4 + 31) / 32, 32 * kRedRows, 0, st>>>(part_w, part_b, nsplit, No, Ni, dW, ldw, db, accumulate);
    DC_LAUNCH_OK();
    return DC_OK;
}

extern "C" int dc_gemm_wgrad_tf32x3(const float *dY, int ldy, const float *X, int ldx, int64_t T, int No, int Ni, float *dW,
                                    int ldw, float *db, int accumulate, void *workspace, dc_stream_t stream) {
    return wgrad_launch<false>(dY, ldy, X, ldx, T, nullptr, nullptr, No, Ni, dW, ldw, db, accumulate, workspace, stream,
                               "dc_gemm_wgrad_tf32x3");
}

extern "C" int dc_gemm_wgrad_tf32x3_rows(const float *dY, int ldy, const float *X, int ldx, const int32_t *x_rows, int64_t T,
                                         const int32_t *t_dev, int No, int Ni, float *dW, int ldw, float *db, int accumulate,
                                         void *workspace, dc_stream_t stream) {
    return wgrad_launch<true>(dY, ldy, X, ldx, T, t_dev, x_rows, No, Ni, dW, ldw, db, accumulate, workspace, stream,
                              "dc_gemm_wgrad_tf32x3_rows");
}

extern "C" int dc_gemm_unit_max(const float *basic, const float *w, const float *bias, float *xmax, float *xmax_copy, int ld_x,
                                uint8_t *argmax, int64_t n_tokens, int n_units, dc_stream_t stream) {
    DC_REQUIRE(basic && w && bias && xmax && argmax && n_tokens > 0, DC_EINVAL, "dc_gemm_unit_max: null pointer / empty input");
    DC_REQUIRE(n_units == 5 || n_units == 16, DC_EUNSUPPORTED, "dc_gemm_unit_max: n_units=%d (5 or 16; 1-unit groups are plain GEMMs)", n_units);
    DC_REQUIRE(ld_x >= BN && n_tokens * n_units < (1ll << 31) - BM, DC_EINVAL, "dc_gemm_unit_max: bad ld_x / size");
    DC_REQUIRE(((uintptr_t)basic & 15) == 0 && ((uintptr_t)w & 15) == 0, DC_EINVAL, "dc_gemm_unit_max: pointers must be 16-byte aligned");
    const int M = (int)(n_tokens * n_units);
    cudaStream_t st = dc_cu_stream(stream);
    if (n_units == 5) return launch_ws<5>(basic, BN, w, BN, bias, xmax, ld_x, M, BN, BN, 0, xmax_copy, argmax, st);
    return launch_ws<16>(basic, BN, w, BN, bias, xmax, ld_x, M, BN, BN, 0, xmax_copy, argmax, st);
}

extern "C" int dc_unit_embed_fwd_mask(const float *units, const float *w_b, const float *b_b, float *basic_out, uint32_t *mask_out,
                                      const float *w, const float *bias, float *xmax, float *xmax_copy, int ld_x, uint8_t *argmax,
                                      int64_t n_tokens, int n_units, dc_stream_t stream) {
    DC_REQUIRE(units && w_b && b_b && w && bias && xmax && n_tokens > 0, DC_EINVAL, "dc_unit_embed_fwd: null pointer / empty input");
    DC_REQUIRE(n_units == 1 || n_units == 5 || n_units == 16, DC_EUNSUPPORTED, "dc_unit_embed_fwd: n_units=%d (1, 5 or 16)", n_units);
    DC_REQUIRE(n_units == 1 ? (argmax == nullptr && xmax_copy == nullptr) : argmax != nullptr, DC_EINVAL,
               "dc_unit_embed_fwd: the arg-max (and the copy) go with the max-pool of n_units 5 and 16 only");
    DC_REQUIRE(ld_x >= BN && ld_x % 4 == 0 && n_tokens * n_units < (1ll << 31) - BM, DC_EINVAL, "dc_unit_embed_fwd: bad ld_x / size");
    DC_REQUIRE(((uintptr_t)units & 15) == 0 && ((uintptr_t)basic_out & 15) == 0 && ((uintptr_t)w & 15) == 0 && ((uintptr_t)bias & 15) == 0 &&
                   ((uintptr_t)xmax & 15) == 0 && ((uintptr_t)xmax_copy & 15) == 0 && ((uintptr_t)mask_out & 15) == 0,
               DC_EINVAL, "dc_unit_embed_fwd: units, basic_out, mask_out, w, bias, xmax, xmax_copy must be 16-byte aligned");
    const int M = (int)(n_tokens * n_units);
    const GenA gen{units, w_b, b_b, basic_out, mask_out};
    cudaStream_t st = dc_cu_stream(stream);
    if (n_units == 1) return launch_ws<0, true>(nullptr, BN, w, BN, bias, xmax, ld_x, M, BN, BN, 0, nullptr, nullptr, st, gen);
    if (n_units == 5) return launch_ws<5, true>(nullptr, BN, w, BN, bias, xmax, ld_x, M, BN, BN, 0, xmax_copy, argmax, st, gen);
    return launch_ws<16, true>(nullptr, BN, w, BN, bias, xmax, ld_x, M, BN, BN, 0, xmax_copy, argmax, st, gen);
}

extern "C" int dc_unit_embed_fwd(const float *units, const float *w_b, const float *b_b, float *basic_out, const float *w, const float *bias,
                                 float *xmax, float *xmax_copy, int ld_x, uint8_t *argmax, int64_t n_tokens, int n_units,
                                 dc_stream_t stream) {
    return dc_unit_embed_fwd_mask(units, w_b, b_b, basic_out, nullptr, w, bias, xmax, xmax_copy, ld_x, argmax, n_tokens, n_units, stream);
}

extern "C" int dc_unit_dgrad_fused_mask(const float *d_xmax, const float *d_xmax2, int ld_dx, const uint8_t *argmax, const float *dlogits,
                                        int ld_dl, const float *att, const float *w_t, const float *units, const uint32_t *mask,
                                        const float *w_b, const float *b_b, int64_t n_tokens, int n_units, float *dw_b, float *db_b,
                                        int accumulate, void *workspace, dc_stream_t stream) {
    DC_REQUIRE(w_t && units && w_b && b_b && dw_b && db_b && workspace && n_tokens > 0, DC_EINVAL, "dc_unit_dgrad_fused: null pointer / empty input");
    DC_REQUIRE(n_units == 1 || n_units == 5 || n_units == 16, DC_EUNSUPPORTED, "dc_unit_dgrad_fused: n_units=%d (1, 5 or 16)", n_units);
    DC_REQUIRE((d_xmax == nullptr && d_xmax2 == nullptr) || (d_xmax != nullptr && ld_dx >= BN && ld_dx % 4 == 0), DC_EINVAL,
               "dc_unit_dgrad_fused: bad d_xmax / ld_dx");
    DC_REQUIRE(d_xmax == nullptr || n_units == 1 || argmax != nullptr, DC_EINVAL, "dc_unit_dgrad_fused: routing needs the arg-max");
    DC_REQUIRE((dlogits == nullptr) == (att == nullptr) && (dlogits == nullptr || ld_dl >= n_units), DC_EINVAL,
               "dc_unit_dgrad_fused: dlogits and att come together");
    DC_REQUIRE(n_tokens * n_units < (1ll << 31) - BM, DC_EINVAL, "dc_unit_dgrad_fused: too many rows");
    DC_REQUIRE(((uintptr_t)d_xmax & 15) == 0 && ((uintptr_t)d_xmax2 & 15) == 0 && ((uintptr_t)argmax & 3) == 0 && ((uintptr_t)att & 15) == 0 &&
                   ((uintptr_t)w_t & 15) == 0 && ((uintptr_t)units & 15) == 0 && ((uintptr_t)mask & 15) == 0 && ((uintptr_t)workspace & 15) == 0,
               DC_EINVAL, "dc_unit_dgrad_fused: d_xmax, att, w_t, units, mask must be 16-byte aligned (arg-max 4-byte)");
    const int n_tok = (int)n_tokens;
    const int tile_rows = BM - BM % n_units;
    int grid = (int)((n_tokens * n_units + tile_rows - 1) / tile_rows);
    if (grid > dc_sm_count()) grid = dc_sm_count();
    float *partial = reinterpret_cast<float *>(workspace);
    cudaStream_t st = dc_cu_stream(stream);
#define DC_LAUNCH_DGRAD(NU, MASK)                                                                                                    \
    do {                                                                                                                              \
        DC_CUDA(cudaFuncSetAttribute(unit_dgrad_kernel<NU, MASK>, cudaFuncAttributeMaxDynamicSharedMemorySize, (int)kDgSmemBytes)); \
        unit_dgrad_kernel<NU, MASK><<<grid, kThreads, kDgSmemBytes, st>>>(d_xmax, d_xmax2, ld_dx, argmax, dlogits, ld_dl, att, w_t,  \
                                                                          units, mask, w_b, b_b, n_tok, partial);                     \
    } while (0)
    if (mask != nullptr) {
        if (n_units == 1) DC_LAUNCH_DGRAD(1, true);
        else if (n_units == 5) DC_LAUNCH_DGRAD(5, true);
        else DC_LAUNCH_DGRAD(16, true);
    } else {
        if (n_units == 1) DC_LAUNCH_DGRAD(1, false);
        else if (n_units == 5) DC_LAUNCH_DGRAD(5, false);
        else DC_LAUNCH_DGRAD(16, false);
    }
#undef DC_LAUNCH_DGRAD
    DC_LAUNCH_OK();
    return dc_unit_basic_reduce(partial, grid, dw_b, db_b, accumulate, st);
}

extern "C" int dc_unit_dgrad_fused(const float *d_xmax, const float *d_xmax2, int ld_dx, const uint8_t *argmax, const float *dlogits,
                                   int ld_dl, const float *att, const float *w_t, const float *units, const float *w_b,
                                   const float *b_b, int64_t n_tokens, int n_units, float *dw_b, float *db_b, int accumulate,
                                   void *workspace, dc_stream_t stream) {
    return dc_unit_dgrad_fused_mask(d_xmax, d_xmax2, ld_dx, argmax, dlogits, ld_dl, att, w_t, units, nullptr, w_b, b_b, n_tokens, n_units,
                                    dw_b, db_b, accumulate, workspace, stream);
}

extern "C" int dc_unit_wgrad_routed(const float *d_xmax, const float *d_xmax2, int ld_dx, const uint8_t *argmax, const float *basic,
                                    int64_t n_tokens, int n_units, float *dW, float *db, void *workspace, dc_stream_t stream) {
    DC_REQUIRE(d_xmax && argmax && basic && dW && db && workspace && n_tokens > 0, DC_EINVAL, "dc_unit_wgrad_routed: null pointer / empty input");
    DC_REQUIRE(n_units == 5 || n_units == 16, DC_EUNSUPPORTED, "dc_unit_wgrad_routed: n_units=%d (5 or 16; a 1-unit group is dc_gemm_wgrad_tf32x3)", n_units);
    DC_REQUIRE(ld_dx >= BM && n_tokens * n_units < (1ll << 31) - BK, DC_EINVAL, "dc_unit_wgrad_routed: bad ld_dx / size");
    DC_REQUIRE(((uintptr_t)basic & 15) == 0 && ((uintptr_t)dW & 15) == 0 && ((uintptr_t)db & 15) == 0 && ((uintptr_t)workspace & 15) == 0,
               DC_EINVAL, "dc_unit_wgrad_routed: pointers must be 16-byte aligned");
    const int No = BM, Ni = BN, nsplit = wgrad_splits(No, Ni);
    const int T = (int)(n_tokens * n_units);
    float *part_w = reinterpret_cast<float *>(workspace);
    float *part_b = part_w + (size_t)nsplit * No * Ni;
    cudaStream_t st = dc_cu_stream(stream);
    if (n_units == 5) {
        DC_CUDA(cudaFuncSetAttribute(gemm_wgrad_kernel<5>, cudaFuncAttributeMaxDynamicSharedMemorySize, (int)kWgSmemBytes));
        gemm_wgrad_kernel<5><<<nsplit, kThreads, kWgSmemBytes, st>>>(d_xmax, ld_dx, d_xmax2, argmax, basic, BN, T, No, Ni, nsplit,
                                                                                part_w, part_b);
    } else {
        DC_CUDA(cudaFuncSetAttribute(gemm_wgrad_kernel<16>, cudaFuncAttributeMaxDynamicSharedMemorySize, (int)kWgSmemBytes));
        gemm_wgrad_kernel<16><<<nsplit, kThreads, kWgSmemBytes, st>>>(d_xmax, ld_dx, d_xmax2, argmax, basic, BN, T, No, Ni, nsplit,
                                                                                 part_w, part_b);
    }
    DC_LAUNCH_OK();
    wgrad_reduce_kernel<<<(BM * BN / 4 + No / 4 + 31) / 32, 32 * kRedRows, 0, st>>>(part_w, part_b, nsplit, No, Ni, dW, Ni, db, 0);
    DC_LAUNCH_OK();
    return DC_OK;
}
```

dotaclient_b200/encoder_ops.py:

```python
import torch

from . import _lib
from .ops import PROFILE, _f32c, _need_cuda, _u8, gemm_tf32x3, gemm_wgrad_supported, gemm_wgrad_tf32x3

UNITS = (1, 5, 16, 16, 1, 1)
OFFSETS = (0, 1, 6, 22, 38, 39)
MAX_UNITS = 40
C = 128
XCAT = 7 * C

_basic_ws = {}


def _basic_workspace(device):
    ws = _basic_ws.get(device)
    if ws is None:
        ws = torch.empty(int(_lib.load().dc_unit_basic_bwd_workspace_bytes()), dtype=torch.uint8, device=device)
        _basic_ws[device] = ws
    return ws


_env_ws = {}


def _env_workspace(device):
    ws = _env_ws.get(device)
    if ws is None:
        ws = torch.empty(int(_lib.load().dc_env_bwd_workspace_bytes()), dtype=torch.uint8, device=device)
        _env_ws[device] = ws
    return ws


_wgrad_ws = {}


def _wgrad_workspace(No, Ni, device):
    key = (No, Ni, device)
    ws = _wgrad_ws.get(key)
    if ws is None:
        ws = torch.empty(int(_lib.load().dc_gemm_wgrad_workspace_bytes(No, Ni)), dtype=torch.uint8, device=device)
        _wgrad_ws[key] = ws
    return ws




def _ptr(t, float_offset=0):
    return t.data_ptr() + 4 * float_offset


def _ptr6(tensors):
    return (_lib._c.c_void_p * 6)(*[t.data_ptr() for t in tensors])


class UnitEncoder(torch.autograd.Function):

    @staticmethod
    def forward(ctx, link, wait, need_grad, env, w_e, b_e, w_b, b_b, *rest):
        units, weights, biases = rest[:6], rest[6:12], rest[12:18]
        ctx.link = link
        _need_cuda(env, w_b, *units)
        lib = _lib.load()
        st = _lib.stream_ptr()
        lead = units[0].shape[:-2]
        N = 1
        for d in lead:
            N *= d
        dev = units[0].device
        w_b, b_b = _f32c(w_b.detach()), _f32c(b_b.detach())
        units = [_f32c(u.detach()).reshape(N * n, 12) for u, n in zip(units, UNITS)]
        units = [u if u.data_ptr() % 16 == 0 else u.clone() for u in units]
        weights = [_f32c(w.detach()) for w in weights]
        biases = [_f32c(b.detach()) for b in biases]
        xcat = torch.empty((N, XCAT), dtype=torch.float32, device=dev)
        argmax = torch.zeros((5, N, C), dtype=torch.uint8, device=dev)
        env2 = _f32c(env.detach()).reshape(N, 3)
        w_e, b_e = _f32c(w_e.detach()), _f32c(b_e.detach())
        if wait is not None:
            wait(env2)
        with PROFILE.span("env_fwd", 1, 4 * N * (3 + C)):
            _lib.check(lib.dc_env_fwd(env2.data_ptr(), w_e.data_ptr(), b_e.data_ptr(), xcat.data_ptr(), XCAT, N, st), "dc_env_fwd")
        basics, masks = [], []
        for g, n_u in enumerate(UNITS):
            R = N * n_u
            if wait is not None:
                wait(units[g])
            if g == 5:
                continue
            basic = torch.empty((R, C), dtype=torch.float32, device=dev) if need_grad else None
            mask = torch.empty((R, 4), dtype=torch.int32, device=dev) if need_grad else None
            copy = _ptr(xcat, 6 * C) if g == 3 else None
            am = argmax[g].data_ptr() if n_u > 1 else None
            nbytes = 4 * (R * 12 + (R * C + R * 4 if need_grad else 0) + C * C + N * C) + (N * C if n_u > 1 else 0)
            with PROFILE.span("gemm_unit_max" if n_u > 1 else "gemm_tf32x3", 1, nbytes):
                _lib.check(lib.dc_unit_embed_fwd_mask(units[g].data_ptr(), w_b.data_ptr(), b_b.data_ptr(), _lib.ptr(basic), _lib.ptr(mask),
                                                      weights[g].data_ptr(), biases[g].data_ptr(), _ptr(xcat, (g + 1) * C), copy, XCAT,
                                                      am, N, n_u, st), "dc_unit_embed_fwd_mask")
            basics.append(basic)
            masks.append(mask)
        link["units"], link["w_b"], link["b_b"] = units, w_b, b_b
        link["weights"], link["biases"] = weights, biases
        ctx.N = N
        ctx.lead = lead
        ctx.save_for_backward(argmax, *units, *basics, *weights, env2, xcat, w_b, b_b, *masks)
        return xcat.view(*lead, XCAT)

    @staticmethod
    def backward(ctx, d_xcat):
        saved = ctx.saved_tensors
        argmax, units, basics, weights, env2, xcat = saved[0], saved[1:7], saved[7:12], saved[12:18], saved[18], saved[19]
        w_b, b_b, masks = saved[20], saved[21], saved[22:27]
        N = ctx.N
        lib = _lib.load()
        st = _lib.stream_ptr()
        dev = argmax.device
        pending = ctx.link.pop("pending", None)
        d_xcat = _f32c(d_xcat).reshape(N, XCAT)
        dw_e = torch.empty((C, 3), dtype=torch.float32, device=dev)
        db_e = torch.empty(C, dtype=torch.float32, device=dev)
        with PROFILE.span("env_bwd", 2, 4 * N * (2 * C + 3)):
            _lib.check(lib.dc_env_bwd(d_xcat.data_ptr(), xcat.data_ptr(), XCAT, env2.data_ptr(), dw_e.data_ptr(), db_e.data_ptr(),
                                      N, _env_workspace(dev).data_ptr(), st), "dc_env_bwd")
        dl = att = s_head = att_head = count = None
        if pending is not None:
            dl, att, s_head, att_head, count = pending
        dw_b = torch.empty((C, 12), dtype=torch.float32, device=dev)
        db_b = torch.empty(C, dtype=torch.float32, device=dev)
        dw_all = torch.zeros((6, C, C), dtype=torch.float32, device=dev)
        db_all = torch.zeros((6, C), dtype=torch.float32, device=dev)
        ws_w = _wgrad_workspace(C, C, dev)
        ws_b = _basic_workspace(dev)
        for g, (n_u, off) in enumerate(zip(UNITS, OFFSETS)):
            R = N * n_u
            routed = g < 5
            dx = _ptr(d_xcat, (g + 1) * C) if routed else None
            dx2 = _ptr(d_xcat, 6 * C) if g == 3 else None
            if routed and n_u > 1:
                with PROFILE.span("gemm_wgrad", 2, 4 * (R * C + C * C + N * C) + N * C):
                    _lib.check(lib.dc_unit_wgrad_routed(dx, dx2, XCAT, argmax[g].data_ptr(), basics[g].data_ptr(), N, n_u,
                                                        dw_all[g].data_ptr(), db_all[g].data_ptr(), ws_w.data_ptr(), st),
                               "dc_unit_wgrad_routed")
            elif routed:
                with PROFILE.span("gemm_wgrad", 2, 4 * (2 * R * C + C * C)):
                    _lib.check(lib.dc_gemm_wgrad_tf32x3(dx, XCAT, basics[g].data_ptr(), C, R, C, C, dw_all[g].data_ptr(), C,
                                                        db_all[g].data_ptr(), 0, ws_w.data_ptr(), st), "dc_gemm_wgrad_tf32x3")
            wt = weights[g].t().contiguous()
            mask = masks[g] if routed else None
            with PROFILE.span("unit_dgrad_fused", 2, N * (4 * C + C) * (1 if routed else 0) + 4 * R * 12 + (16 * R if routed else 0)
                              + (4 * N * (C + n_u) if dl is not None else 0)):
                _lib.check(lib.dc_unit_dgrad_fused_mask(dx, dx2, XCAT, argmax[g].data_ptr() if (routed and n_u > 1) else None,
                                                        None if dl is None else _ptr(dl, off), MAX_UNITS, None if att is None else att.data_ptr(),
                                                        wt.data_ptr(), units[g].data_ptr(), _lib.ptr(mask), w_b.data_ptr(), b_b.data_ptr(),
                                                        N, n_u, dw_b.data_ptr(), db_b.data_ptr(), 1 if g > 0 else 0, ws_b.data_ptr(), st),
                           "dc_unit_dgrad_fused_mask")
        if dl is not None:
            dw_head, _ = gemm_wgrad_tf32x3(att_head, s_head, want_bias=False, t_dev=count, t_host=ctx.link.get("n_active"))
            dw_all += dw_head[:, :6 * C].reshape(C, 6, C).permute(1, 0, 2)
            db_all += dw_head[:, 6 * C:6 * C + 6].t()
        dws, dbs = list(dw_all.unbind(0)), list(db_all.unbind(0))
        return (None, None, None, None, dw_e, db_e, dw_b, db_b) + (None,) * 6 + tuple(dws) + tuple(dbs)


QW = 7 * C


class TargetUnit(torch.autograd.Function):

    @staticmethod
    def forward(ctx, att, link):
        _need_cuda(att)
        units, w_b, b_b = link["units"], link["w_b"], link["b_b"]
        lead = att.shape[:-1]
        N = att.numel() // C
        att2 = _f32c(att.detach()).reshape(N, C)
        dev = att2.device
        bm = _head_matrix(link)
        q = gemm_tf32x3(att2, bm.t().contiguous())
        logits = torch.empty((N, MAX_UNITS), dtype=torch.float32, device=dev)
        with PROFILE.span("target_unit_fwd", 1, 4 * N * (MAX_UNITS * 12 + QW + MAX_UNITS)):
            _lib.check(_lib.load().dc_target_unit_q_fwd(q.data_ptr(), QW, _ptr6(units), w_b.data_ptr(), b_b.data_ptr(),
                                                        logits.data_ptr(), N, _lib.stream_ptr()), "dc_target_unit_q_fwd")
        ctx.save_for_backward(att2, bm, w_b, b_b, *units)
        ctx.link = link
        ctx.att_shape = att.shape
        return logits.view(*lead, MAX_UNITS)

    @staticmethod
    def backward(ctx, dlogits):
        att2, bm, w_b, b_b = ctx.saved_tensors[:4]
        units = ctx.saved_tensors[4:]
        N = att2.shape[0]
        dl = _f32c(dlogits).reshape(N, MAX_UNITS)
        s = torch.empty((N, QW), dtype=torch.float32, device=att2.device)
        with PROFILE.span("target_unit_bwd", 1):
            _lib.check(_lib.load().dc_target_unit_q_bwd(dl.data_ptr(), _ptr6(units), w_b.data_ptr(), b_b.data_ptr(), s.data_ptr(),
                                                        QW, N, _lib.stream_ptr()), "dc_target_unit_q_bwd")
        d_att = gemm_tf32x3(s, bm)
        ctx.link["pending"] = (dl, att2, s, att2, None)
        return d_att.view(ctx.att_shape), None


def _head_matrix(link):
    bias_block = torch.zeros((C, C), dtype=torch.float32, device=link["w_b"].device)
    bias_block[:, :6] = torch.stack(link["biases"], dim=1)
    return torch.cat(list(link["weights"]) + [bias_block], dim=1)


_rows_ws = {}


def target_rows(mask, action):
    _need_cuda(mask, action)
    m, a = _u8(mask).reshape(-1, MAX_UNITS), _u8(action).reshape(-1, MAX_UNITS)
    N = m.shape[0]
    dev = m.device
    ws = _rows_ws.get((N, dev))
    if ws is None:
        ws = _rows_ws[(N, dev)] = torch.empty(int(_lib.load().dc_target_rows_workspace_bytes(N)), dtype=torch.uint8, device=dev)
    rows = torch.empty(N, dtype=torch.int32, device=dev)
    count = torch.empty(1, dtype=torch.int32, device=dev)
    flags = torch.empty(N, dtype=torch.uint8, device=dev)
    with PROFILE.span("target_rows", 2, 2 * N * MAX_UNITS + 2 * N + 4 * N):
        _lib.check(_lib.load().dc_target_rows(m.data_ptr(), a.data_ptr(), N, rows.data_ptr(), count.data_ptr(), flags.data_ptr(),
                                              ws.data_ptr(), _lib.stream_ptr()), "dc_target_rows")
    return rows, count, flags


def _gemm_rows(a, b, rows, count, n_host, bias=None, gather=False, out=None, out_rows=None):
    M = rows.numel()
    K, N = a.shape[1], b.shape[0]
    ld = (out if out is not None else out_rows).stride(0)
    n = M if n_host is None else n_host
    with PROFILE.span("gemm_tf32x3", 1, 4 * (n * K + N * K + n * N * ((out is not None) + (out_rows is not None)))):
        _lib.check(_lib.load().dc_gemm_tf32x3_rows(a.data_ptr(), a.stride(0), b.data_ptr(), b.stride(0), _lib.ptr(bias), _lib.ptr(out),
                                                   _lib.ptr(out_rows), ld, M, count.data_ptr(), rows.data_ptr(), 1 if gather else 0,
                                                   N, K, 0, _lib.stream_ptr()), "dc_gemm_tf32x3_rows")


def _zero_inactive(flags, dst, n_host):
    N, width = dst.shape
    n = 0 if n_host is None else N - n_host
    with PROFILE.span("rows_zero", 1, N + 4 * n * width):
        _lib.check(_lib.load().dc_rows_zero_inactive(flags.data_ptr(), N, dst.data_ptr(), dst.stride(0), width, _lib.stream_ptr()),
                   "dc_rows_zero_inactive")


class TargetUnitRows(torch.autograd.Function):

    @staticmethod
    def forward(ctx, y, w_att, b_att, link, rows, count, flags):
        _need_cuda(y, rows, count)
        units, w_b, b_b = link["units"], link["w_b"], link["b_b"]
        H = y.shape[-1]
        lead = y.shape[:-1]
        N = y.numel() // H
        dev = y.device
        n_act = int(count.item()) if PROFILE.enabled else None
        link["n_active"] = n_act
        y2 = _f32c(y.detach()).reshape(N, H)
        w_att, b_att = _f32c(w_att.detach()), _f32c(b_att.detach())
        att_c = torch.empty((N, C), dtype=torch.float32, device=dev)
        att = torch.empty((N, C), dtype=torch.float32, device=dev)
        _gemm_rows(y2, w_att, rows, count, n_act, bias=b_att, gather=True, out=att_c, out_rows=att)
        _zero_inactive(flags, att, n_act)
        bm = _head_matrix(link)
        q_c = torch.empty((N, QW), dtype=torch.float32, device=dev)
        _gemm_rows(att_c, bm.t().contiguous(), rows, count, n_act, out=q_c)
        logits = torch.empty((N, MAX_UNITS), dtype=torch.float32, device=dev)
        _zero_inactive(flags, logits, n_act)
        nb = N if n_act is None else n_act
        with PROFILE.span("target_unit_fwd", 1, 4 * nb * (MAX_UNITS * 12 + QW + MAX_UNITS)):
            _lib.check(_lib.load().dc_target_unit_q_fwd_rows(q_c.data_ptr(), QW, _ptr6(units), w_b.data_ptr(), b_b.data_ptr(),
                                                             logits.data_ptr(), N, rows.data_ptr(), count.data_ptr(),
                                                             _lib.stream_ptr()), "dc_target_unit_q_fwd_rows")
        ctx.save_for_backward(y2, att_c, att, w_att, bm, w_b, b_b, rows, count, flags, *units)
        ctx.link = link
        ctx.n_act = n_act
        ctx.y_shape = y.shape
        return logits.view(*lead, MAX_UNITS)

    @staticmethod
    def backward(ctx, dlogits):
        y2, att_c, att, w_att, bm, w_b, b_b, rows, count, flags = ctx.saved_tensors[:10]
        units = ctx.saved_tensors[10:]
        N, H = y2.shape
        n_act = ctx.n_act
        nb = N if n_act is None else n_act
        dev = y2.device
        dl = _f32c(dlogits).reshape(N, MAX_UNITS)
        s_c = torch.empty((N, QW), dtype=torch.float32, device=dev)
        with PROFILE.span("target_unit_bwd", 1, 4 * nb * (MAX_UNITS * 12 + MAX_UNITS + QW)):
            _lib.check(_lib.load().dc_target_unit_q_bwd_rows(dl.data_ptr(), _ptr6(units), w_b.data_ptr(), b_b.data_ptr(),
                                                             s_c.data_ptr(), QW, N, rows.data_ptr(), count.data_ptr(),
                                                             _lib.stream_ptr()), "dc_target_unit_q_bwd_rows")
        d_att_c = torch.empty((N, C), dtype=torch.float32, device=dev)
        _gemm_rows(s_c, bm, rows, count, n_act, out=d_att_c)
        dy = dw = db = None
        if ctx.needs_input_grad[0]:
            dy = torch.empty((N, H), dtype=torch.float32, device=dev)
            _gemm_rows(d_att_c, w_att.t().contiguous(), rows, count, n_act, out_rows=dy)
            _zero_inactive(flags, dy, n_act)
            dy = dy.view(ctx.y_shape)
        if ctx.needs_input_grad[1] or ctx.needs_input_grad[2]:
            dw, db = gemm_wgrad_tf32x3(d_att_c, y2, want_bias=True, t_dev=count, t_host=n_act, x_rows=rows)
        ctx.link["pending"] = (dl, att, s_c, att_c, count)
        return dy, dw, db, None, None, None, None


def unit_encoder(env, w_e, b_e, w_b, b_b, units, weights, biases, wait=None):
    link = {}
    tensors = (env, w_e, b_e, w_b, b_b, *units, *weights, *biases)
    need_grad = torch.is_grad_enabled() and any(t.requires_grad for t in tensors)
    xcat = UnitEncoder.apply(link, wait, need_grad, *tensors)
    return link, xcat


def target_unit(att, link):
    return TargetUnit.apply(att, link)


def target_unit_rows(y, w_att, b_att, link, rows, count, flags):
    return TargetUnitRows.apply(y, w_att, b_att, link, rows, count, flags)


__all__ = ["unit_encoder", "target_unit", "target_unit_rows", "target_rows", "gemm_wgrad_supported"]
```

include/dotaclient_b200.h:

```cpp
#ifndef DOTACLIENT_B200_H
#define DOTACLIENT_B200_H

#include <stddef.h>
#include <stdint.h>

#ifdef __cplusplus
extern "C" {
#endif

#define DC_OK 0
#define DC_EINVAL (-1)
#define DC_EUNSUPPORTED (-2)

#define DC_CELL_GRU 0
#define DC_CELL_LSTM 1

#define DC_NUM_HEADS 5
#define DC_LOSS_SLOTS 16

typedef void *dc_stream_t;

int dc_version(void);
const char *dc_last_error(void);
int dc_device_info(int *sm_count, int *cc_major, int *cc_minor);

int dc_gae_scan(const float *rewards, int n_sub, const float *values, const int64_t *seg_off,
                int n_seg, const float *boot_value, const float *boot_reward, double gamma,
                double lam, float *adv, float *ret, dc_stream_t stream);

#define DC_VTRACE_STATS_SLOTS 8
int dc_vtrace_scan(const float *rewards, int n_sub, const float *values, const float *logp_target,
                   const float *logp_behaviour, const int64_t *seg_off, int n_seg, const int64_t *valid_len,
                   const float *boot_value, double gamma, double lam, double rho_clip, double c_clip, float *pg_adv,
                   float *vs, double *seg_stats, dc_stream_t stream);

int dc_gae_scan_indexed(const float *rewards, int n_sub, const float *values, int64_t ld_values, const int64_t *tok,
                        const int64_t *seg_off, int n_seg, const float *boot_value, const float *boot_reward,
                        double gamma, double lam, float *adv, float *ret, dc_stream_t stream);
int dc_vtrace_scan_indexed(const float *rewards, int n_sub, const float *values, int64_t ld_values,
                           const float *logp_target, const float *logp_behaviour, const int64_t *tok,
                           const int64_t *seg_off, int n_seg, const int64_t *valid_len, const float *boot_value,
                           double gamma, double lam, double rho_clip, double c_clip, float *pg_adv, float *vs,
                           double *seg_stats, dc_stream_t stream);

#define DC_UPGO_STATS_SLOTS 3
int dc_upgo_scan(const float *rewards, int n_sub, const float *values, const float *logp_target,
                 const float *logp_behaviour, const int64_t *seg_off, int n_seg, const int64_t *valid_len,
                 const float *boot_value, double gamma, double rho_clip, double coef, float *adv, double *seg_stats,
                 dc_stream_t stream);
int dc_upgo_scan_indexed(const float *rewards, int n_sub, const float *values, int64_t ld_values,
                         const float *logp_target, const float *logp_behaviour, const int64_t *tok,
                         const int64_t *seg_off, int n_seg, const int64_t *valid_len, const float *boot_value,
                         double gamma, double rho_clip, double coef, float *adv, double *seg_stats, dc_stream_t stream);

#define DC_VALUE_HEADS_MAX 10
int dc_gae_scan_heads(const float *rewards, int n_sub, const int32_t *group, int K, const float *values,
                      const int64_t *seg_off, int n_seg, const float *boot_value, const float *boot_reward,
                      const double *gammas, double lam, float *adv, float *ret, dc_stream_t stream);
int dc_gae_scan_heads_indexed(const float *rewards, int n_sub, const int32_t *group, int K, const float *values,
                              int64_t ld_values, const int64_t *tok, const int64_t *seg_off, int n_seg,
                              const float *boot_value, const float *boot_reward, const double *gammas, double lam,
                              float *adv, float *ret, dc_stream_t stream);

#define DC_VALUE_HEADS_STATS_SLOTS 20
#define DC_VALUE_HEADS_WORKSPACE_BYTES 131072
int dc_value_heads_loss(const float *value, int64_t ld_value, const float *ret, const float *old_value,
                        const uint8_t *valid, int64_t N, int K, const double *hparams, float *dvalue, int64_t ld_dvalue,
                        float *out, float *stats, float *head_stats, void *workspace, dc_stream_t stream);

typedef struct {
    const void *src;
    void *dst;
    int64_t outer;
    int64_t src_cols;
    int64_t row_bytes;
} dc_gather_desc;
#define DC_GATHER_MAX_TENSORS 32
int dc_gather_columns(const dc_gather_desc *descs, int n_desc, const int64_t *index, int64_t n_index,
                      dc_stream_t stream);
int dc_gather_columns_fill(const dc_gather_desc *descs, int n_desc, const int64_t *index, int64_t n_index,
                           dc_stream_t stream);

#define DC_REFRESH_MAX_LAYERS 16
int dc_refresh_states(int n_layers, int H, const float *const *h_bufs, const float *const *c_bufs, int64_t R, int64_t t0,
                      const int64_t *step, const int64_t *rollout, const int64_t *slot, int64_t n, int64_t B, int64_t K,
                      float *h0, float *c0, float *reset_h, float *reset_c, double *partial, double *acc,
                      dc_stream_t stream);

size_t dc_rnn_workspace_bytes(int cell, int B, int H);
int dc_rnn_seq_fwd(int cell, float *gates, const float *w_hh, const float *b_hh, float *ybuf,
                   float *cbuf, int B, int S, int H, void *workspace, dc_stream_t stream);
int dc_rnn_seq_bwd(int cell, float *gates, const float *w_hh, const float *ybuf, float *cbuf,
                   const float *dy, const float *dhn, const float *dcn, float *dh0, float *dc0,
                   int B, int S, int H, void *workspace, dc_stream_t stream);

int dc_rnn_seq_fwd_reset(int cell, float *gates, const float *w_hh, const float *b_hh, float *ybuf, float *cbuf,
                         const int32_t *reset_slot, const float *reset_prev, const float *reset_pre, int K,
                         int B, int S, int H, void *workspace, dc_stream_t stream);
int dc_rnn_seq_bwd_reset(int cell, float *gates, const float *w_hh, const float *ybuf, float *cbuf,
                         const float *dy, const float *dhn, const float *dcn, float *dh0, float *dc0,
                         const int32_t *reset_slot, const float *reset_prev, int K,
                         int B, int S, int H, void *workspace, dc_stream_t stream);

int dc_gemm_tf32x3_supported(int64_t M, int N, int K);
int dc_gemm_tf32x3(const float *A, int lda, const float *B, int ldb, const float *bias, float *C, int ldc,
                   int64_t M, int N, int K, int relu, dc_stream_t stream);

size_t dc_gemm_wgrad_workspace_bytes(int No, int Ni);
int dc_gemm_wgrad_tf32x3(const float *dY, int ldy, const float *X, int ldx, int64_t T, int No, int Ni,
                         float *dW, int ldw, float *db, int accumulate, void *workspace, dc_stream_t stream);
int dc_gemm_tf32x3_rows(const float *A, int lda, const float *B, int ldb, const float *bias, float *C, float *C_rows, int ldc,
                        int64_t M, const int32_t *count, const int32_t *rows, int gather_a, int N, int K, int relu, dc_stream_t stream);
int dc_gemm_wgrad_tf32x3_rows(const float *dY, int ldy, const float *X, int ldx, const int32_t *x_rows, int64_t T, const int32_t *t_dev,
                              int No, int Ni, float *dW, int ldw, float *db, int accumulate, void *workspace, dc_stream_t stream);

size_t dc_unit_basic_bwd_workspace_bytes(void);
int dc_env_fwd(const float *env, const float *w_e, const float *b_e, float *out, int ld_out, int64_t N,
               dc_stream_t stream);
size_t dc_env_bwd_workspace_bytes(void);
int dc_env_bwd(const float *d_out, const float *out, int ld, const float *env, float *dw_e, float *db_e, int64_t N,
               void *workspace, dc_stream_t stream);
int dc_gemm_unit_max(const float *basic, const float *w, const float *bias, float *xmax, float *xmax_copy, int ld_x,
                     uint8_t *argmax, int64_t n_tokens, int n_units, dc_stream_t stream);
int dc_unit_embed_fwd(const float *units, const float *w_b, const float *b_b, float *basic_out, const float *w, const float *bias,
                      float *xmax, float *xmax_copy, int ld_x, uint8_t *argmax, int64_t n_tokens, int n_units, dc_stream_t stream);
int dc_unit_embed_fwd_mask(const float *units, const float *w_b, const float *b_b, float *basic_out, uint32_t *mask_out, const float *w,
                           const float *bias, float *xmax, float *xmax_copy, int ld_x, uint8_t *argmax, int64_t n_tokens, int n_units,
                           dc_stream_t stream);
int dc_target_unit_q_fwd(const float *q, int ld_q, const float *const units[6], const float *w_b, const float *b_b, float *logits,
                         int64_t N, dc_stream_t stream);
int dc_target_unit_q_bwd(const float *dlogits, const float *const units[6], const float *w_b, const float *b_b, float *s, int ld_s,
                         int64_t N, dc_stream_t stream);
int dc_target_unit_q_fwd_rows(const float *q, int ld_q, const float *const units[6], const float *w_b, const float *b_b, float *logits,
                              int64_t N, const int32_t *rows, const int32_t *count, dc_stream_t stream);
int dc_target_unit_q_bwd_rows(const float *dlogits, const float *const units[6], const float *w_b, const float *b_b, float *s, int ld_s,
                              int64_t N, const int32_t *rows, const int32_t *count, dc_stream_t stream);
size_t dc_target_rows_workspace_bytes(int64_t N);
int dc_target_rows(const uint8_t *mask, const uint8_t *action, int64_t N, int32_t *rows, int32_t *count, uint8_t *flags,
                   void *workspace, dc_stream_t stream);
int dc_rows_zero_inactive(const uint8_t *flags, int64_t N, float *dst, int ld, int width, dc_stream_t stream);
int dc_unit_wgrad_routed(const float *d_xmax, const float *d_xmax2, int ld_dx, const uint8_t *argmax, const float *basic,
                         int64_t n_tokens, int n_units, float *dW, float *db, void *workspace, dc_stream_t stream);
int dc_unit_dgrad_fused(const float *d_xmax, const float *d_xmax2, int ld_dx, const uint8_t *argmax, const float *dlogits,
                        int ld_dl, const float *att, const float *w_t, const float *units, const float *w_b,
                        const float *b_b, int64_t n_tokens, int n_units, float *dw_b, float *db_b, int accumulate,
                        void *workspace, dc_stream_t stream);
int dc_unit_dgrad_fused_mask(const float *d_xmax, const float *d_xmax2, int ld_dx, const uint8_t *argmax, const float *dlogits,
                             int ld_dl, const float *att, const float *w_t, const float *units, const uint32_t *mask, const float *w_b,
                             const float *b_b, int64_t n_tokens, int n_units, float *dw_b, float *db_b, int accumulate,
                             void *workspace, dc_stream_t stream);

#define DC_PPO_WORKSPACE_BYTES 512
int dc_ppo_loss_fwd_bwd(const float *const logits[DC_NUM_HEADS],
                        const uint8_t *const masks[DC_NUM_HEADS],
                        const uint8_t *const actions[DC_NUM_HEADS], const float *old_logp,
                        const float *adv_raw, const float *ret, const float *value, int64_t N,
                        float e_clip, float entropy_coef, float vf_coef,
                        float *const dlogits[DC_NUM_HEADS], float *dvalue, float *out,
                        int32_t *n_actions, void *workspace, dc_stream_t stream);

int dc_ppo_loss_fwd_bwd_strided(const float *const logits[DC_NUM_HEADS], const int64_t ld_logits[DC_NUM_HEADS],
                                const uint8_t *const masks[DC_NUM_HEADS],
                                const uint8_t *const actions[DC_NUM_HEADS], const float *old_logp,
                                const float *adv_raw, const float *ret, const float *value, int64_t ld_value,
                                int64_t N, float e_clip, float entropy_coef, float vf_coef,
                                float *const dlogits[DC_NUM_HEADS], const int64_t ld_dlogits[DC_NUM_HEADS],
                                float *dvalue, int64_t ld_dvalue, float *out, int32_t *n_actions,
                                void *workspace, dc_stream_t stream);

#define DC_HPARAM_SLOTS 10
#define DC_HP_LR 0
#define DC_HP_E_CLIP 1
#define DC_HP_ENTROPY_COEF 2
#define DC_HP_VF_COEF 3
#define DC_HP_MAX_GRAD_NORM 4
#define DC_HP_VALUE_CLIP 5
#define DC_HP_VALUE_NORM_MEAN 6
#define DC_HP_VALUE_NORM_STD 7
#define DC_HP_KL_COEF 8
#define DC_HP_KL_STOP 9

#define DC_PPO_STATS_SLOTS 24
#define DC_STAT_APPROX_KL 0
#define DC_STAT_CLIP_FRACTION 6
#define DC_STAT_EXPLAINED_VAR 12
#define DC_STAT_JOINT_APPROX_KL 13
#define DC_STAT_JOINT_CLIP_FRACTION 14
#define DC_STAT_KL 16
#define DC_STAT_KL_PENALTY 22
int dc_ppo_loss_fwd_bwd_dev(const float *const logits[DC_NUM_HEADS], const int64_t ld_logits[DC_NUM_HEADS],
                            const uint8_t *const masks[DC_NUM_HEADS],
                            const uint8_t *const actions[DC_NUM_HEADS], const float *old_logp,
                            const float *adv_raw, const float *ret, const float *value, int64_t ld_value,
                            const float *old_value, int64_t N, const double *hparams,
                            float *const dlogits[DC_NUM_HEADS], const int64_t ld_dlogits[DC_NUM_HEADS],
                            float *dvalue, int64_t ld_dvalue, float *out, float *stats, int32_t *n_actions,
                            void *workspace, dc_stream_t stream);

int dc_ppo_loss_fwd_bwd_masked(const float *const logits[DC_NUM_HEADS], const int64_t ld_logits[DC_NUM_HEADS],
                               const uint8_t *const masks[DC_NUM_HEADS],
                               const uint8_t *const actions[DC_NUM_HEADS], const float *old_logp,
                               const float *adv_raw, const float *ret, const float *value, int64_t ld_value,
                               const float *old_value, const uint8_t *valid, int64_t N, const double *hparams,
                               float *const dlogits[DC_NUM_HEADS], const int64_t ld_dlogits[DC_NUM_HEADS],
                               float *dvalue, int64_t ld_dvalue, float *out, float *stats, int32_t *n_actions,
                               void *workspace, dc_stream_t stream);

int dc_ppo_loss_fwd_bwd_joint(const float *const logits[DC_NUM_HEADS], const int64_t ld_logits[DC_NUM_HEADS],
                              const uint8_t *const masks[DC_NUM_HEADS],
                              const uint8_t *const actions[DC_NUM_HEADS], const float *old_logp,
                              const float *adv_raw, const float *ret, const float *value, int64_t ld_value,
                              const float *old_value, const uint8_t *valid, int64_t N, const double *hparams,
                              float *const dlogits[DC_NUM_HEADS], const int64_t ld_dlogits[DC_NUM_HEADS],
                              float *dvalue, int64_t ld_dvalue, float *out, float *stats, int32_t *n_actions,
                              void *workspace, dc_stream_t stream);

#define DC_KL_ROW_FLOATS 65
int dc_selected_logp_rows(const float *const logits[DC_NUM_HEADS], const uint8_t *const masks[DC_NUM_HEADS],
                          const uint8_t *const actions[DC_NUM_HEADS], int64_t N, float *logp_out, float *logp_rows,
                          dc_stream_t stream);
int dc_ppo_loss_fwd_bwd_kl(const float *const logits[DC_NUM_HEADS], const int64_t ld_logits[DC_NUM_HEADS],
                           const uint8_t *const masks[DC_NUM_HEADS], const uint8_t *const actions[DC_NUM_HEADS],
                           const float *old_logp, const float *old_log_probs, const float *adv_raw, const float *ret,
                           const float *value, int64_t ld_value, const float *old_value, const uint8_t *valid, int64_t N,
                           const double *hparams, int joint, float *const dlogits[DC_NUM_HEADS],
                           const int64_t ld_dlogits[DC_NUM_HEADS], float *dvalue, int64_t ld_dvalue, float *out,
                           float *stats, float *kl_out, int32_t *n_actions, void *workspace, dc_stream_t stream);

#define DC_TEACHER_STATS_SLOTS 7
int dc_ppo_loss_fwd_bwd_teacher(const float *const logits[DC_NUM_HEADS], const int64_t ld_logits[DC_NUM_HEADS],
                                const uint8_t *const masks[DC_NUM_HEADS], const uint8_t *const actions[DC_NUM_HEADS],
                                const float *old_logp, const float *old_log_probs, const float *teacher_log_probs,
                                const float *adv_raw, const float *ret, const float *value, int64_t ld_value,
                                const float *old_value, const uint8_t *valid, int64_t N, const double *hparams,
                                const double *teacher_coef, int joint, float *const dlogits[DC_NUM_HEADS],
                                const int64_t ld_dlogits[DC_NUM_HEADS], float *dvalue, int64_t ld_dvalue, float *out,
                                float *stats, float *kl_out, float *teacher_stats, int32_t *n_actions, void *workspace,
                                dc_stream_t stream);

#define DC_BC_STATS_SLOTS 12
int dc_ppo_loss_fwd_bwd_bc(const float *const logits[DC_NUM_HEADS], const int64_t ld_logits[DC_NUM_HEADS],
                           const uint8_t *const masks[DC_NUM_HEADS], const uint8_t *const actions[DC_NUM_HEADS],
                           const float *adv_raw, const float *ret, const float *value, int64_t ld_value,
                           const float *old_value, const uint8_t *valid, int64_t N, const double *hparams,
                           float *const dlogits[DC_NUM_HEADS], const int64_t ld_dlogits[DC_NUM_HEADS], float *dvalue,
                           int64_t ld_dvalue, float *out, float *stats, float *bc_stats, int32_t *n_actions,
                           void *workspace, dc_stream_t stream);

#define DC_DUAL_CLIP_STATS_SLOTS 7
int dc_ppo_loss_fwd_bwd_dual_clip(const float *const logits[DC_NUM_HEADS], const int64_t ld_logits[DC_NUM_HEADS],
                                  const uint8_t *const masks[DC_NUM_HEADS], const uint8_t *const actions[DC_NUM_HEADS],
                                  const float *old_logp, const float *old_log_probs, const float *teacher_log_probs,
                                  const float *adv_raw, const float *ret, const float *value, int64_t ld_value,
                                  const float *old_value, const uint8_t *valid, int64_t N, const double *hparams,
                                  const double *teacher_coef, const double *dual_clip, int joint,
                                  float *const dlogits[DC_NUM_HEADS], const int64_t ld_dlogits[DC_NUM_HEADS],
                                  float *dvalue, int64_t ld_dvalue, float *out, float *stats, float *kl_out,
                                  float *teacher_stats, float *dual_clip_stats, int32_t *n_actions, void *workspace,
                                  dc_stream_t stream);

int dc_value_norm_stats(const float *x, const uint8_t *valid, int64_t N, double *out, dc_stream_t stream);
int dc_value_denorm(const float *v, int64_t ld_v, int64_t N, double mu, double sigma, float *out, dc_stream_t stream);
int dc_value_head_rescale(float *w, int64_t n, float *b, double mu_old, double sigma_old, double mu_new, double sigma_new,
                          dc_stream_t stream);

int dc_selected_logp(const float *const logits[DC_NUM_HEADS],
                     const uint8_t *const masks[DC_NUM_HEADS],
                     const uint8_t *const actions[DC_NUM_HEADS], int64_t N, float *logp_out,
                     dc_stream_t stream);

int dc_grad_flags(float *flat_grad, int64_t total, const int32_t *seg_head, int n_seg,
                  const int32_t *n_actions, dc_stream_t stream);
int dc_grad_finish(float *flat_param, float *flat_grad, float *exp_avg, float *exp_avg_sq,
                   int32_t *steps, const int64_t *seg_lo, const int64_t *seg_hi, const int32_t *seg_head, int n_seg,
                   int64_t total, double lr, double beta1, double beta2, double adam_eps,
                   double max_norm, const float *loss_out, float *metrics, void *workspace,
                   dc_stream_t stream);
int dc_grad_finish_dev(float *flat_param, float *flat_grad, float *exp_avg, float *exp_avg_sq,
                       int32_t *steps, const int64_t *seg_lo, const int64_t *seg_hi, const int32_t *seg_head, int n_seg,
                       int64_t total, const double *hparams, double beta1, double beta2, double adam_eps,
                       const float *loss_out, float *metrics, void *workspace, dc_stream_t stream);
#define DC_FINISH_WORKSPACE_BYTES 1024
#define DC_FINISH_KL_METRICS 6
int dc_grad_finish_kl(float *flat_param, float *flat_grad, float *exp_avg, float *exp_avg_sq,
                      int32_t *steps, const int64_t *seg_lo, const int64_t *seg_hi, const int32_t *seg_head, int n_seg,
                      int64_t total, const double *hparams, double beta1, double beta2, double adam_eps,
                      const float *loss_out, float *metrics, void *workspace, dc_stream_t stream);

int dc_select_actions(const float *const logits[DC_NUM_HEADS], const int64_t ld[DC_NUM_HEADS],
                      const uint8_t *const masks[DC_NUM_HEADS], const float *u, int64_t A, int32_t *chosen,
                      float *logp, dc_stream_t stream);

#ifdef __cplusplus
}
#endif
#endif
```

Baseline: 89.99.

## Use split-FP16 wgmma with per-column scaling for routed unit weight gradient

Replaces the TF32x3 routed unit weight-gradient GEMM with a split-FP16 (hi/lo, three-product) wgmma kernel that uses k16 MMAs and half-width operand tiles. Per-column power-of-two scales are derived from column maxima: the forward embedding kernel accumulates activation column maxima via atomics, and a new small kernel computes dY column maxima before backward. The aim is to halve the shared-memory traffic per operand and raise tensor-core throughput while keeping near-FP32 accuracy. It adds an extra colmax pass and a memset, and its accuracy depends on the scaling keeping values within FP16 range.

```diff
diff --git a/dotaclient_b200/_lib.py b/dotaclient_b200/_lib.py
--- a/dotaclient_b200/_lib.py
+++ b/dotaclient_b200/_lib.py
@@ -49,12 +49,15 @@
     "dc_env_bwd_workspace_bytes": (_sz, []),
     "dc_env_bwd": (_i32, [_vp, _vp, _i32, _vp, _vp, _vp, _i64, _vp, _vp]),
     "dc_unit_wgrad_routed": (_i32, [_vp, _vp, _i32, _vp, _vp, _i64, _i32, _vp, _vp, _vp, _vp]),
+    "dc_unit_wgrad_routed_f16": (_i32, [_vp, _vp, _i32, _vp, _vp, _i64, _i32, _vp, _vp, _vp, _vp, _vp, _vp]),
+    "dc_unit_dy_colmax": (_i32, [_vp, _vp, _i32, _i32, _i64, _vp, _vp]),
     "dc_unit_dgrad_fused": (_i32, [_vp, _vp, _i32, _vp, _vp, _i32, _vp, _vp, _vp, _vp, _vp, _i64, _i32, _vp, _vp, _i32, _vp, _vp]),
     "dc_unit_dgrad_fused_mask": (_i32, [_vp, _vp, _i32, _vp, _vp, _i32, _vp, _vp, _vp, _vp, _vp, _vp, _i64, _i32, _vp, _vp, _i32, _vp,
                                         _vp]),
     "dc_gemm_unit_max": (_i32, [_vp, _vp, _vp, _vp, _vp, _i32, _vp, _i64, _i32, _vp]),
     "dc_unit_embed_fwd": (_i32, [_vp, _vp, _vp, _vp, _vp, _vp, _vp, _vp, _i32, _vp, _i64, _i32, _vp]),
     "dc_unit_embed_fwd_mask": (_i32, [_vp, _vp, _vp, _vp, _vp, _vp, _vp, _vp, _vp, _i32, _vp, _i64, _i32, _vp]),
+    "dc_unit_embed_fwd_colmax": (_i32, [_vp, _vp, _vp, _vp, _vp, _vp, _vp, _vp, _vp, _vp, _i32, _vp, _i64, _i32, _vp]),
     "dc_target_unit_q_fwd": (_i32, [_vp, _i32, _c.c_void_p * 6, _vp, _vp, _vp, _i64, _vp]),
     "dc_target_unit_q_bwd": (_i32, [_vp, _c.c_void_p * 6, _vp, _vp, _vp, _i32, _i64, _vp]),
     "dc_target_unit_q_fwd_rows": (_i32, [_vp, _i32, _c.c_void_p * 6, _vp, _vp, _vp, _i64, _vp, _vp, _vp]),
diff --git a/dotaclient_b200/csrc/gemm_tf32x3.cu b/dotaclient_b200/csrc/gemm_tf32x3.cu
--- a/dotaclient_b200/csrc/gemm_tf32x3.cu
+++ b/dotaclient_b200/csrc/gemm_tf32x3.cu
@@ -1,3 +1,5 @@
+#include <cuda_fp16.h>
+
 #include "dc_common.cuh"
 #include "unit_basic.cuh"
 
@@ -326,7 +328,7 @@
 struct GenA {
     const float *units, *w_b, *b_b;
     float *basic_out;
-    uint32_t *mask_out;
+    uint32_t *mask_out, *colmax;
 };
 
 __device__ __forceinline__ void cp_async16(uint32_t dst, const void *src, uint32_t src_bytes) {
@@ -363,7 +365,7 @@
     }
 }
 
-template <int NU, bool kGenA, bool kDevM = false>
+template <int NU, bool kGenA, bool kDevM = false, bool kColMax = false>
 __global__ void __launch_bounds__(kWsThreads, 1) gemm_ws_kernel(const float *__restrict__ A, int lda,
                                                                 const float *__restrict__ B, int ldb,
                                                                 const float *__restrict__ bias, float *__restrict__ C,
@@ -412,6 +414,7 @@
             }
         };
         fetch(mb0);
+        float cmax[4] = {0.f, 0.f, 0.f, 0.f};
         uint32_t c = kc;
         for (int mb = mb0; mb < m_blocks; mb += mstride, c += 4) {
             const int m0 = mb * kTileRows;
@@ -432,11 +435,22 @@
                 float4 v = make_float4(dc_unit_basic(u, wb[0], bb[0]), dc_unit_basic(u, wb[1], bb[1]), dc_unit_basic(u, wb[2], bb[2]),
                                        dc_unit_basic(u, wb[3], bb[3]));
                 if (!ok) v = make_float4(0.f, 0.f, 0.f, 0.f);
+                if constexpr (kColMax) {
+                    cmax[0] = fmaxf(cmax[0], v.x); cmax[1] = fmaxf(cmax[1], v.y); cmax[2] = fmaxf(cmax[2], v.z); cmax[3] = fmaxf(cmax[3], v.w);
+                }
                 *reinterpret_cast<float4 *>(chunk + r * 128 + ((ch ^ (r & 7)) << 4)) = v;
                 if (gen.basic_out != nullptr && ok) *reinterpret_cast<float4 *>(gen.basic_out + (size_t)(m0 + r) * BN + j0) = v;
             }
             __syncwarp();
             if (lane == 0) dc_mbar_arrive(&full[s]);
+        }
+        if constexpr (kColMax) {
+#pragma unroll
+            for (int e = 0; e < 4; ++e) {
+                cmax[e] = fmaxf(cmax[e], __shfl_xor_sync(0xffffffffu, cmax[e], 8));
+                cmax[e] = fmaxf(cmax[e], __shfl_xor_sync(0xffffffffu, cmax[e], 16));
+                if (lane < 8) atomicMax(gen.colmax + j0 + e, __float_as_uint(fabsf(cmax[e])));
+            }
         }
         return;
     }
@@ -1072,6 +1086,242 @@
     }
 }
 
+constexpr int kWhK = 64;
+constexpr int kWhStages = 3;
+constexpr int kWhLdX = BN + 4;
+constexpr int kWhTileBytes = BM * kWhK * 2;
+constexpr int kWhStageBytes = 2 * kWhTileBytes + kWhK * kWhLdX * 4;
+constexpr int kWhFlush = kWgFlush * BK / kWhK;
+constexpr size_t kWhOffColsum = (size_t)kWhStages * kWhStageBytes;
+constexpr size_t kWhOffScale = kWhOffColsum + 2 * BM * 4;
+constexpr size_t kWhOffBars = kWhOffScale + BM * 4;
+constexpr size_t kWhSmemBytes = kWhOffBars + 2 * kWhStages * 8 + 1024 ;
+static_assert(kWhStageBytes % 1024 == 0, "the swizzled dY^T tiles need 1024-byte aligned slots");
+static_assert(kWhSmemBytes <= 227 * 1024, "split-FP16 weight-gradient GEMM exceeds the shared-memory opt-in");
+
+__device__ __forceinline__ int f16_scale_exp(uint32_t bits) {
+    bits &= 0x7fffffffu;
+    const int E = (int)(bits >> 23);
+    if (bits == 0 || E == 0xff) return 0;
+    const int fl = E > 0 ? E - 127 : (31 - __clz(bits)) - 149;
+    return min(14 - fl, 126);
+}
+__device__ __forceinline__ float pow2f(int e) { return __uint_as_float((uint32_t)(127 + e) << 23); }
+
+__device__ __forceinline__ void split_f16x2(float x0, float x1, uint32_t &hi, uint32_t &lo) {
+    const __half2 h = __floats2half2_rn(x0, x1);
+    const float2 hf = __half22float2(h);
+    const __half2 l = __floats2half2_rn(x0 - hf.x, x1 - hf.y);
+    hi = *reinterpret_cast<const uint32_t *>(&h);
+    lo = *reinterpret_cast<const uint32_t *>(&l);
+}
+
+#define DC_ACC8(b) "+f"(d[b]), "+f"(d[b + 1]), "+f"(d[b + 2]), "+f"(d[b + 3]), "+f"(d[b + 4]), "+f"(d[b + 5]), "+f"(d[b + 6]), "+f"(d[b + 7])
+__device__ __forceinline__ void wgmma_m64n128k16_f16_rs(float (&d)[64], const uint32_t (&a)[4], uint64_t desc_b) {
+    asm volatile(
+        "{\n\t.reg .pred p;\n\tsetp.ne.b32 p, %69, 0;\n\t"
+        "wgmma.mma_async.sync.aligned.m64n128k16.f32.f16.f16 "
+        "{%0, %1, %2, %3, %4, %5, %6, %7, %8, %9, %10, %11, %12, %13, %14, %15, "
+        "%16, %17, %18, %19, %20, %21, %22, %23, %24, %25, %26, %27, %28, %29, %30, %31, "
+        "%32, %33, %34, %35, %36, %37, %38, %39, %40, %41, %42, %43, %44, %45, %46, %47, "
+        "%48, %49, %50, %51, %52, %53, %54, %55, %56, %57, %58, %59, %60, %61, %62, %63}, "
+        "{%64, %65, %66, %67}, %68, p, 1, 1, 0;\n\t}\n"
+        : DC_ACC8(0), DC_ACC8(8), DC_ACC8(16), DC_ACC8(24), DC_ACC8(32), DC_ACC8(40), DC_ACC8(48), DC_ACC8(56)
+        : "r"(a[0]), "r"(a[1]), "r"(a[2]), "r"(a[3]), "l"(desc_b), "r"(1));
+}
+#undef DC_ACC8
+
+template <int NU>
+__global__ void __launch_bounds__(kThreads, 1) unit_wgrad_f16_kernel(const float *__restrict__ dY, int ldy, const float *__restrict__ dY2,
+                                                                     const uint8_t *__restrict__ argmax, const float *__restrict__ X, int T,
+                                                                     int nsplit, float *__restrict__ part_w, float *__restrict__ part_b,
+                                                                     const uint32_t *__restrict__ x_colmax,
+                                                                     const uint32_t *__restrict__ dy_colmax) {
+    constexpr int kTPC = kWhK / NU;
+    constexpr int kRPC = kTPC * NU;
+    extern __shared__ unsigned char smem_raw[];
+    unsigned char *ring = smem_base(smem_raw);
+    float *colsum_s = reinterpret_cast<float *>(ring + kWhOffColsum);
+    float *inv_o = reinterpret_cast<float *>(ring + kWhOffScale);
+    uint64_t *full = reinterpret_cast<uint64_t *>(ring + kWhOffBars), *empty = full + kWhStages;
+
+    const int warp = threadIdx.x >> 5, lane = threadIdx.x & 31;
+    const int split = blockIdx.x;
+    const int chunks_total = (T + kRPC - 1) / kRPC;
+    const int my_chunks = split < chunks_total ? (chunks_total - split + nsplit - 1) / nsplit : 0;
+    if (threadIdx.x == 0) {
+        for (int s = 0; s < kWhStages; ++s) { dc_mbar_init(&full[s], kProducerThreads + 4); dc_mbar_init(&empty[s], kConsumerThreads / 32); }
+        asm volatile("fence.mbarrier_init.release.cluster;" ::: "memory");
+    }
+    if (threadIdx.x < BM) inv_o[threadIdx.x] = pow2f(-f16_scale_exp(__ldg(dy_colmax + threadIdx.x)));
+    __syncthreads();
+
+    if (warp < kConsumerWarp0) {
+        const int g = warp >> 2, t = threadIdx.x & (kProducerThreads - 1), xc = t & 31;
+        const float so = pow2f(f16_scale_exp(__ldg(dy_colmax + t)));
+        float cs = 0.f, cc = 0.f;
+        for (int j = g; j < my_chunks; j += kProducerGroups) {
+            const int tok0 = (split + j * nsplit) * kTPC, n_tok = T / NU;
+            float dv[kTPC];
+            int am[kTPC];
+#pragma unroll
+            for (int k = 0; k < kTPC; ++k) {
+                const bool ok = tok0 + k < n_tok;
+                const size_t at = (size_t)(tok0 + k) * ldy + t;
+                dv[k] = ok ? __ldg(dY + at) : 0.f;
+                if (ok && dY2 != nullptr) dv[k] += __ldg(dY2 + at);
+                am[k] = ok ? (int)__ldg(argmax + (size_t)(tok0 + k) * 128 + t) : 255;
+            }
+            float sc = 0.f;
+            uint16_t hb[kTPC], lb[kTPC];
+#pragma unroll
+            for (int k = 0; k < kTPC; ++k) {
+                sc += am[k] < NU ? dv[k] : 0.f;
+                const float x = dv[k] * so;
+                const __half h = __float2half_rn(x), l = __float2half_rn(x - __half2float(h));
+                hb[k] = __half_as_ushort(h);
+                lb[k] = __half_as_ushort(l);
+            }
+            const float y = sc - cc, cs_new = cs + y;
+            cc = (cs_new - cs) - y;
+            cs = cs_new;
+            const int t0 = (split + j * nsplit) * kRPC, tend = min(T, t0 + kRPC);
+            const int s = j % kWhStages;
+            dc_mbar_wait(&empty[s], ((j / kWhStages) & 1) ^ 1);
+            unsigned char *st = ring + (size_t)s * kWhStageBytes;
+            const uint32_t xs = dc_smem_u32(st + 2 * kWhTileBytes);
+#pragma unroll
+            for (int r = 0; r < kWhK / 4; ++r) {
+                const int row = (t >> 5) + 4 * r;
+                const bool ok = t0 + row < tend;
+                cp_async16(xs + (row * kWhLdX + 4 * xc) * 4, X + (ok ? (size_t)(t0 + row) * BN + 4 * xc : 0), ok ? 16u : 0u);
+            }
+            cp_async_arrive(&full[s]);
+#pragma unroll
+            for (int c = 0; c < kWhK / 8; ++c) {
+                uint32_t hw[4], lw[4];
+#pragma unroll
+                for (int p = 0; p < 4; ++p) {
+                    const int i0 = 8 * c + 2 * p, i1 = i0 + 1;
+                    const bool r0 = i0 < kRPC && am[i0 / NU] == i0 % NU, r1 = i1 < kRPC && am[i1 / NU] == i1 % NU;
+                    hw[p] = (r0 ? (uint32_t)hb[i0 / NU] : 0u) | ((r1 ? (uint32_t)hb[i1 / NU] : 0u) << 16);
+                    lw[p] = (r0 ? (uint32_t)lb[i0 / NU] : 0u) | ((r1 ? (uint32_t)lb[i1 / NU] : 0u) << 16);
+                }
+                const int off = t * 128 + ((c ^ (t & 7)) << 4);
+                *reinterpret_cast<uint4 *>(st + off) = make_uint4(hw[0], hw[1], hw[2], hw[3]);
+                *reinterpret_cast<uint4 *>(st + kWhTileBytes + off) = make_uint4(lw[0], lw[1], lw[2], lw[3]);
+            }
+            asm volatile("fence.proxy.async.shared::cta;" ::: "memory");
+            __syncwarp();
+            if (lane == 0) dc_mbar_arrive(&full[s]);
+        }
+        colsum_s[g * 128 + t] = cs;
+        asm volatile("cp.async.wait_all;" ::: "memory");
+    } else {
+        const int ct = threadIdx.x - kConsumerWarp0 * 32, wg = ct >> 7, w4 = (ct >> 5) & 3, q = lane & 3;
+        const int rlo = 64 * wg + 16 * w4 + (lane >> 2);
+        const int e_lo = f16_scale_exp(__ldg(x_colmax + rlo)), e_hi = f16_scale_exp(__ldg(x_colmax + rlo + 8));
+        const float s_lo = pow2f(e_lo), s_hi = pow2f(e_hi), i_lo = pow2f(-e_lo), i_hi = pow2f(-e_hi);
+        float d[64];
+#pragma unroll
+        for (int i = 0; i < 64; ++i) d[i] = 0.f;
+        uint32_t ahi[2][4] = {}, alo[2][4] = {};
+#pragma unroll
+        for (int i = 0; i < 64; ++i) dc_reg_fence(d[i]);
+        float *pt = part_w + (size_t)split * BM * BN + ct * 4;
+        const auto flush = [&](bool add) {
+            dc_wgmma_wait0();
+#pragma unroll
+            for (int k = 0; k < 64; ++k) dc_reg_fence(d[k]);
+#pragma unroll
+            for (int m = 0; m < 16; ++m) {
+                const float2 io = *reinterpret_cast<const float2 *>(inv_o + 8 * m + 2 * q);
+                const float4 v = make_float4(d[4 * m] * i_lo * io.x, d[4 * m + 1] * i_lo * io.y, d[4 * m + 2] * i_hi * io.x,
+                                             d[4 * m + 3] * i_hi * io.y);
+                if (add)
+                    asm volatile("red.global.add.v4.f32 [%0], {%1, %2, %3, %4};" ::"l"(pt + m * kConsumerThreads * 4), "f"(v.x), "f"(v.y),
+                                 "f"(v.z), "f"(v.w) : "memory");
+                else
+                    *reinterpret_cast<float4 *>(pt + m * kConsumerThreads * 4) = v;
+            }
+#pragma unroll
+            for (int k = 0; k < 64; ++k) d[k] = 0.f;
+#pragma unroll
+            for (int k = 0; k < 64; ++k) dc_reg_fence(d[k]);
+        };
+        int j = 0;
+        do {
+            const int j_end = min(my_chunks, j + kWhFlush);
+            for (; j < j_end; ++j) {
+                const int s = j % kWhStages;
+                dc_mbar_wait(&full[s], (j / kWhStages) & 1);
+                const uint32_t st = dc_smem_u32(ring + (size_t)s * kWhStageBytes);
+                const uint32_t xk = st + 2 * kWhTileBytes + (2 * q * kWhLdX + rlo) * 4;
+                const uint64_t b_hi = dc_wgmma_desc(st), b_lo = dc_wgmma_desc(st + kWhTileBytes);
+#pragma unroll
+                for (int ks = 0; ks < kWhK / 16; ++ks) {
+                    const int b = ks & 1;
+                    const uint32_t x16 = xk + 16 * ks * kWhLdX * 4;
+#pragma unroll
+                    for (int e = 0; e < 4; ++e) {
+                        const uint32_t xa = x16 + ((e >> 1) * 8 * kWhLdX + (e & 1) * 8) * 4;
+                        const float sx = (e & 1) ? s_hi : s_lo;
+                        split_f16x2(lds_f32(xa) * sx, lds_f32(xa + kWhLdX * 4) * sx, ahi[b][e], alo[b][e]);
+                    }
+                    dc_wgmma_fence();
+                    const uint64_t adv = (uint64_t)(ks * 2);
+                    wgmma_m64n128k16_f16_rs(d, ahi[b], b_lo + adv);
+                    wgmma_m64n128k16_f16_rs(d, alo[b], b_hi + adv);
+                    wgmma_m64n128k16_f16_rs(d, ahi[b], b_hi + adv);
+                    dc_wgmma_commit();
+                    wgmma_wait1();
+#pragma unroll
+                    for (int e = 0; e < 4; ++e) asm volatile("" : "+r"(ahi[b ^ 1][e]), "+r"(alo[b ^ 1][e])::"memory");
+                    if (ks == 0 && j > 0) {
+                        __syncwarp();
+                        if (lane == 0) dc_mbar_arrive(&empty[(j - 1) % kWhStages]);
+                    }
+                }
+            }
+            flush(j > kWhFlush);
+        } while (j < my_chunks);
+    }
+    __syncthreads();
+    if (part_b != nullptr && threadIdx.x < 128)
+        part_b[(size_t)split * BM + threadIdx.x] = colsum_s[threadIdx.x] + colsum_s[128 + threadIdx.x];
+}
+
+constexpr int kCmRows = 8;
+__global__ void __launch_bounds__(32 * kCmRows) unit_dy_colmax_kernel(const float *__restrict__ dY, const float *__restrict__ dY2, int ld,
+                                                                     int n_tok, uint32_t *__restrict__ colmax) {
+    __shared__ uint4 sh[kCmRows][32];
+    const int x = threadIdx.x & 31, y = threadIdx.x >> 5, slot = blockIdx.y;
+    dY += BM * slot;
+    colmax += BM * slot;
+    if (slot + 1 < (int)gridDim.y) dY2 = nullptr;
+    uint4 m = make_uint4(0u, 0u, 0u, 0u);
+#pragma unroll 4
+    for (int n = blockIdx.x * kCmRows + y; n < n_tok; n += gridDim.x * kCmRows) {
+        float4 v = __ldg(reinterpret_cast<const float4 *>(dY + (size_t)n * ld) + x);
+        if (dY2 != nullptr) {
+            const float4 v2 = __ldg(reinterpret_cast<const float4 *>(dY2 + (size_t)n * ld) + x);
+            v.x += v2.x; v.y += v2.y; v.z += v2.z; v.w += v2.w;
+        }
+        m.x = max(m.x, __float_as_uint(fabsf(v.x))); m.y = max(m.y, __float_as_uint(fabsf(v.y)));
+        m.z = max(m.z, __float_as_uint(fabsf(v.z))); m.w = max(m.w, __float_as_uint(fabsf(v.w)));
+    }
+    sh[y][x] = m;
+    __syncthreads();
+    if (y == 0) {
+#pragma unroll
+        for (int r = 1; r < kCmRows; ++r) {
+            m.x = max(m.x, sh[r][x].x); m.y = max(m.y, sh[r][x].y); m.z = max(m.z, sh[r][x].z); m.w = max(m.w, sh[r][x].w);
+        }
+        atomicMax(colmax + 4 * x, m.x); atomicMax(colmax + 4 * x + 1, m.y);
+        atomicMax(colmax + 4 * x + 2, m.z); atomicMax(colmax + 4 * x + 3, m.w);
+    }
+}
+
 }
 
 extern "C" int dc_gemm_tf32x3_supported(int64_t M, int N, int K) { return M > 0 && N > 0 && K > 0 && N % 32 == 0 && K % BK == 0; }
@@ -1081,7 +1331,7 @@
     float *C_rows;
 };
 
-template <int NU, bool kGenA = false, bool kDevM = false>
+template <int NU, bool kGenA = false, bool kDevM = false, bool kColMax = false>
 static int launch_ws(const float *A, int lda, const float *B, int ldb, const float *bias, float *C, int ldc, int M, int N,
                      int K, int relu, float *C_copy, uint8_t *argmax, cudaStream_t st, GenA gen = GenA{}, RowList rl = RowList{}) {
     const int tile_rows = NU == 5 ? 60 : kWsRows;
@@ -1090,8 +1340,8 @@
     if (per_block < 1) per_block = 1;
     if (per_block > m_blocks) per_block = m_blocks;
     const size_t smem = kGenA ? kWsGenSmemBytes : kWsSmemBytes;
-    DC_CUDA(cudaFuncSetAttribute(gemm_ws_kernel<NU, kGenA, kDevM>, cudaFuncAttributeMaxDynamicSharedMemorySize, (int)smem));
-    gemm_ws_kernel<NU, kGenA, kDevM><<<n_blocks * per_block, kWsThreads, smem, st>>>(A, lda, B, ldb, bias, C, ldc, M, N, K, relu, C_copy,
+    DC_CUDA(cudaFuncSetAttribute(gemm_ws_kernel<NU, kGenA, kDevM, kColMax>, cudaFuncAttributeMaxDynamicSharedMemorySize, (int)smem));
+    gemm_ws_kernel<NU, kGenA, kDevM, kColMax><<<n_blocks * per_block, kWsThreads, smem, st>>>(A, lda, B, ldb, bias, C, ldc, M, N, K, relu, C_copy,
                                                                                     argmax, gen, rl.count, rl.a_rows, rl.rows, rl.C_rows);
     DC_LAUNCH_OK();
     return DC_OK;
@@ -1222,9 +1472,9 @@
     return launch_ws<16>(basic, BN, w, BN, bias, xmax, ld_x, M, BN, BN, 0, xmax_copy, argmax, st);
 }
 
-extern "C" int dc_unit_embed_fwd_mask(const float *units, const float *w_b, const float *b_b, float *basic_out, uint32_t *mask_out,
-                                      const float *w, const float *bias, float *xmax, float *xmax_copy, int ld_x, uint8_t *argmax,
-                                      int64_t n_tokens, int n_units, dc_stream_t stream) {
+extern "C" int dc_unit_embed_fwd_colmax(const float *units, const float *w_b, const float *b_b, float *basic_out, uint32_t *mask_out,
+                                        uint32_t *colmax, const float *w, const float *bias, float *xmax, float *xmax_copy, int ld_x,
+                                        uint8_t *argmax, int64_t n_tokens, int n_units, dc_stream_t stream) {
     DC_REQUIRE(units && w_b && b_b && w && bias && xmax && n_tokens > 0, DC_EINVAL, "dc_unit_embed_fwd: null pointer / empty input");
     DC_REQUIRE(n_units == 1 || n_units == 5 || n_units == 16, DC_EUNSUPPORTED, "dc_unit_embed_fwd: n_units=%d (1, 5 or 16)", n_units);
     DC_REQUIRE(n_units == 1 ? (argmax == nullptr && xmax_copy == nullptr) : argmax != nullptr, DC_EINVAL,
@@ -1233,12 +1483,25 @@
     DC_REQUIRE(((uintptr_t)units & 15) == 0 && ((uintptr_t)basic_out & 15) == 0 && ((uintptr_t)w & 15) == 0 && ((uintptr_t)bias & 15) == 0 &&
                    ((uintptr_t)xmax & 15) == 0 && ((uintptr_t)xmax_copy & 15) == 0 && ((uintptr_t)mask_out & 15) == 0,
                DC_EINVAL, "dc_unit_embed_fwd: units, basic_out, mask_out, w, bias, xmax, xmax_copy must be 16-byte aligned");
+    DC_REQUIRE(colmax == nullptr || n_units > 1, DC_EINVAL, "dc_unit_embed_fwd: column maxima go with the max-pool of n_units 5 and 16");
+    DC_REQUIRE(((uintptr_t)colmax & 3) == 0, DC_EINVAL, "dc_unit_embed_fwd: colmax must be 4-byte aligned");
     const int M = (int)(n_tokens * n_units);
-    const GenA gen{units, w_b, b_b, basic_out, mask_out};
+    const GenA gen{units, w_b, b_b, basic_out, mask_out, colmax};
     cudaStream_t st = dc_cu_stream(stream);
     if (n_units == 1) return launch_ws<0, true>(nullptr, BN, w, BN, bias, xmax, ld_x, M, BN, BN, 0, nullptr, nullptr, st, gen);
-    if (n_units == 5) return launch_ws<5, true>(nullptr, BN, w, BN, bias, xmax, ld_x, M, BN, BN, 0, xmax_copy, argmax, st, gen);
+    if (n_units == 5) {
+        if (colmax != nullptr) return launch_ws<5, true, false, true>(nullptr, BN, w, BN, bias, xmax, ld_x, M, BN, BN, 0, xmax_copy, argmax, st, gen);
+        return launch_ws<5, true>(nullptr, BN, w, BN, bias, xmax, ld_x, M, BN, BN, 0, xmax_copy, argmax, st, gen);
+    }
+    if (colmax != nullptr) return launch_ws<16, true, false, true>(nullptr, BN, w, BN, bias, xmax, ld_x, M, BN, BN, 0, xmax_copy, argmax, st, gen);
     return launch_ws<16, true>(nullptr, BN, w, BN, bias, xmax, ld_x, M, BN, BN, 0, xmax_copy, argmax, st, gen);
+}
+
+extern "C" int dc_unit_embed_fwd_mask(const float *units, const float *w_b, const float *b_b, float *basic_out, uint32_t *mask_out,
+                                      const float *w, const float *bias, float *xmax, float *xmax_copy, int ld_x, uint8_t *argmax,
+                                      int64_t n_tokens, int n_units, dc_stream_t stream) {
+    return dc_unit_embed_fwd_colmax(units, w_b, b_b, basic_out, mask_out, nullptr, w, bias, xmax, xmax_copy, ld_x, argmax, n_tokens,
+                                    n_units, stream);
 }
 
 extern "C" int dc_unit_embed_fwd(const float *units, const float *w_b, const float *b_b, float *basic_out, const float *w, const float *bias,
@@ -1322,3 +1585,47 @@
     DC_LAUNCH_OK();
     return DC_OK;
 }
+
+extern "C" int dc_unit_wgrad_routed_f16(const float *d_xmax, const float *d_xmax2, int ld_dx, const uint8_t *argmax, const float *basic,
+                                        int64_t n_tokens, int n_units, float *dW, float *db, void *workspace, const uint32_t *x_colmax,
+                                        const uint32_t *dy_colmax, dc_stream_t stream) {
+    DC_REQUIRE(d_xmax && argmax && basic && dW && db && workspace && x_colmax && dy_colmax && n_tokens > 0, DC_EINVAL,
+               "dc_unit_wgrad_routed_f16: null pointer / empty input");
+    DC_REQUIRE(n_units == 5 || n_units == 16, DC_EUNSUPPORTED, "dc_unit_wgrad_routed_f16: n_units=%d (5 or 16)", n_units);
+    DC_REQUIRE(ld_dx >= BM && n_tokens * n_units < (1ll << 31) - kWhK, DC_EINVAL, "dc_unit_wgrad_routed_f16: bad ld_dx / size");
+    DC_REQUIRE(((uintptr_t)basic & 15) == 0 && ((uintptr_t)dW & 15) == 0 && ((uintptr_t)db & 15) == 0 && ((uintptr_t)workspace & 15) == 0 &&
+                   ((uintptr_t)x_colmax & 3) == 0 && ((uintptr_t)dy_colmax & 3) == 0,
+               DC_EINVAL, "dc_unit_wgrad_routed_f16: pointers must be 16-byte aligned (column maxima 4-byte)");
+    const int No = BM, Ni = BN, nsplit = wgrad_splits(No, Ni);
+    const int T = (int)(n_tokens * n_units);
+    float *part_w = reinterpret_cast<float *>(workspace);
+    float *part_b = part_w + (size_t)nsplit * No * Ni;
+    cudaStream_t st = dc_cu_stream(stream);
+    if (n_units == 5) {
+        DC_CUDA(cudaFuncSetAttribute(unit_wgrad_f16_kernel<5>, cudaFuncAttributeMaxDynamicSharedMemorySize, (int)kWhSmemBytes));
+        unit_wgrad_f16_kernel<5><<<nsplit, kThreads, kWhSmemBytes, st>>>(d_xmax, ld_dx, d_xmax2, argmax, basic, T, nsplit, part_w, part_b,
+                                                                        x_colmax, dy_colmax);
+    } else {
+        DC_CUDA(cudaFuncSetAttribute(unit_wgrad_f16_kernel<16>, cudaFuncAttributeMaxDynamicSharedMemorySize, (int)kWhSmemBytes));
+        unit_wgrad_f16_kernel<16><<<nsplit, kThreads, kWhSmemBytes, st>>>(d_xmax, ld_dx, d_xmax2, argmax, basic, T, nsplit, part_w, part_b,
+                                                                         x_colmax, dy_colmax);
+    }
+    DC_LAUNCH_OK();
+    wgrad_reduce_kernel<<<(BM * BN / 4 + No / 4 + 31) / 32, 32 * kRedRows, 0, st>>>(part_w, part_b, nsplit, No, Ni, dW, Ni, db, 0);
+    DC_LAUNCH_OK();
+    return DC_OK;
+}
+
+extern "C" int dc_unit_dy_colmax(const float *d_xmax, const float *d_xmax2, int ld_dx, int n_slots, int64_t n_tokens, uint32_t *colmax,
+                                 dc_stream_t stream) {
+    DC_REQUIRE(d_xmax && colmax && n_tokens > 0 && n_tokens < (1ll << 31), DC_EINVAL, "dc_unit_dy_colmax: null pointer / bad size");
+    DC_REQUIRE(n_slots >= 1 && n_slots <= 8 && ld_dx >= BM * n_slots && ld_dx % 4 == 0 && ((uintptr_t)d_xmax & 15) == 0 && ((uintptr_t)d_xmax2 & 15) == 0 && ((uintptr_t)colmax & 3) == 0,
+               DC_EINVAL, "dc_unit_dy_colmax: bad ld_dx / alignment");
+    cudaStream_t st = dc_cu_stream(stream);
+    DC_CUDA(cudaMemsetAsync(colmax, 0, (size_t)n_slots * BM * sizeof(uint32_t), st));
+    long long grid = (n_tokens + kCmRows - 1) / kCmRows;
+    if (grid * n_slots > 8ll * dc_sm_count()) grid = (8ll * dc_sm_count() + n_slots - 1) / n_slots;
+    unit_dy_colmax_kernel<<<dim3((unsigned)grid, (unsigned)n_slots), 32 * kCmRows, 0, st>>>(d_xmax, d_xmax2, ld_dx, (int)n_tokens, colmax);
+    DC_LAUNCH_OK();
+    return DC_OK;
+}
diff --git a/dotaclient_b200/encoder_ops.py b/dotaclient_b200/encoder_ops.py
--- a/dotaclient_b200/encoder_ops.py
+++ b/dotaclient_b200/encoder_ops.py
@@ -81,6 +81,7 @@
         with PROFILE.span("env_fwd", 1, 4 * N * (3 + C)):
             _lib.check(lib.dc_env_fwd(env2.data_ptr(), w_e.data_ptr(), b_e.data_ptr(), xcat.data_ptr(), XCAT, N, st), "dc_env_fwd")
         basics, masks = [], []
+        colmax = torch.zeros((3, C), dtype=torch.int32, device=dev) if need_grad else None
         for g, n_u in enumerate(UNITS):
             R = N * n_u
             if wait is not None:
@@ -93,23 +94,24 @@
             am = argmax[g].data_ptr() if n_u > 1 else None
             nbytes = 4 * (R * 12 + (R * C + R * 4 if need_grad else 0) + C * C + N * C) + (N * C if n_u > 1 else 0)
             with PROFILE.span("gemm_unit_max" if n_u > 1 else "gemm_tf32x3", 1, nbytes):
-                _lib.check(lib.dc_unit_embed_fwd_mask(units[g].data_ptr(), w_b.data_ptr(), b_b.data_ptr(), _lib.ptr(basic), _lib.ptr(mask),
-                                                      weights[g].data_ptr(), biases[g].data_ptr(), _ptr(xcat, (g + 1) * C), copy, XCAT,
-                                                      am, N, n_u, st), "dc_unit_embed_fwd_mask")
+                cm = colmax[g - 1].data_ptr() if need_grad and n_u > 1 else None
+                _lib.check(lib.dc_unit_embed_fwd_colmax(units[g].data_ptr(), w_b.data_ptr(), b_b.data_ptr(), _lib.ptr(basic), _lib.ptr(mask),
+                                                        cm, weights[g].data_ptr(), biases[g].data_ptr(), _ptr(xcat, (g + 1) * C), copy,
+                                                        XCAT, am, N, n_u, st), "dc_unit_embed_fwd_colmax")
             basics.append(basic)
             masks.append(mask)
         link["units"], link["w_b"], link["b_b"] = units, w_b, b_b
         link["weights"], link["biases"] = weights, biases
         ctx.N = N
         ctx.lead = lead
-        ctx.save_for_backward(argmax, *units, *basics, *weights, env2, xcat, w_b, b_b, *masks)
+        ctx.save_for_backward(argmax, *units, *basics, *weights, env2, xcat, w_b, b_b, *masks, colmax)
         return xcat.view(*lead, XCAT)
 
     @staticmethod
     def backward(ctx, d_xcat):
         saved = ctx.saved_tensors
         argmax, units, basics, weights, env2, xcat = saved[0], saved[1:7], saved[7:12], saved[12:18], saved[18], saved[19]
-        w_b, b_b, masks = saved[20], saved[21], saved[22:27]
+        w_b, b_b, masks, colmax = saved[20], saved[21], saved[22:27], saved[27]
         N = ctx.N
         lib = _lib.load()
         st = _lib.stream_ptr()
@@ -130,6 +132,10 @@
         db_all = torch.zeros((6, C), dtype=torch.float32, device=dev)
         ws_w = _wgrad_workspace(C, C, dev)
         ws_b = _basic_workspace(dev)
+        dy_colmax = torch.empty((3, C), dtype=torch.int32, device=dev)
+        with PROFILE.span("gemm_wgrad", 2, 4 * N * 4 * C):
+            _lib.check(lib.dc_unit_dy_colmax(_ptr(d_xcat, 2 * C), _ptr(d_xcat, 6 * C), XCAT, 3, N, dy_colmax.data_ptr(), st),
+                       "dc_unit_dy_colmax")
         for g, (n_u, off) in enumerate(zip(UNITS, OFFSETS)):
             R = N * n_u
             routed = g < 5
@@ -137,9 +143,10 @@
             dx2 = _ptr(d_xcat, 6 * C) if g == 3 else None
             if routed and n_u > 1:
                 with PROFILE.span("gemm_wgrad", 2, 4 * (R * C + C * C + N * C) + N * C):
-                    _lib.check(lib.dc_unit_wgrad_routed(dx, dx2, XCAT, argmax[g].data_ptr(), basics[g].data_ptr(), N, n_u,
-                                                        dw_all[g].data_ptr(), db_all[g].data_ptr(), ws_w.data_ptr(), st),
-                               "dc_unit_wgrad_routed")
+                    _lib.check(lib.dc_unit_wgrad_routed_f16(dx, dx2, XCAT, argmax[g].data_ptr(), basics[g].data_ptr(), N, n_u,
+                                                            dw_all[g].data_ptr(), db_all[g].data_ptr(), ws_w.data_ptr(),
+                                                            colmax[g - 1].data_ptr(), dy_colmax[g - 1].data_ptr(), st),
+                               "dc_unit_wgrad_routed_f16")
             elif routed:
                 with PROFILE.span("gemm_wgrad", 2, 4 * (2 * R * C + C * C)):
                     _lib.check(lib.dc_gemm_wgrad_tf32x3(dx, XCAT, basics[g].data_ptr(), C, R, C, C, dw_all[g].data_ptr(), C,
diff --git a/include/dotaclient_b200.h b/include/dotaclient_b200.h
--- a/include/dotaclient_b200.h
+++ b/include/dotaclient_b200.h
@@ -127,6 +127,9 @@
 int dc_unit_embed_fwd_mask(const float *units, const float *w_b, const float *b_b, float *basic_out, uint32_t *mask_out, const float *w,
                            const float *bias, float *xmax, float *xmax_copy, int ld_x, uint8_t *argmax, int64_t n_tokens, int n_units,
                            dc_stream_t stream);
+int dc_unit_embed_fwd_colmax(const float *units, const float *w_b, const float *b_b, float *basic_out, uint32_t *mask_out,
+                             uint32_t *colmax, const float *w, const float *bias, float *xmax, float *xmax_copy, int ld_x,
+                             uint8_t *argmax, int64_t n_tokens, int n_units, dc_stream_t stream);
 int dc_target_unit_q_fwd(const float *q, int ld_q, const float *const units[6], const float *w_b, const float *b_b, float *logits,
                          int64_t N, dc_stream_t stream);
 int dc_target_unit_q_bwd(const float *dlogits, const float *const units[6], const float *w_b, const float *b_b, float *s, int ld_s,
@@ -141,6 +144,11 @@
 int dc_rows_zero_inactive(const uint8_t *flags, int64_t N, float *dst, int ld, int width, dc_stream_t stream);
 int dc_unit_wgrad_routed(const float *d_xmax, const float *d_xmax2, int ld_dx, const uint8_t *argmax, const float *basic,
                          int64_t n_tokens, int n_units, float *dW, float *db, void *workspace, dc_stream_t stream);
+int dc_unit_wgrad_routed_f16(const float *d_xmax, const float *d_xmax2, int ld_dx, const uint8_t *argmax, const float *basic,
+                             int64_t n_tokens, int n_units, float *dW, float *db, void *workspace, const uint32_t *x_colmax,
+                             const uint32_t *dy_colmax, dc_stream_t stream);
+int dc_unit_dy_colmax(const float *d_xmax, const float *d_xmax2, int ld_dx, int n_slots, int64_t n_tokens, uint32_t *colmax,
+                      dc_stream_t stream);
 int dc_unit_dgrad_fused(const float *d_xmax, const float *d_xmax2, int ld_dx, const uint8_t *argmax, const float *dlogits,
                         int ld_dl, const float *att, const float *w_t, const float *units, const float *w_b,
                         const float *b_b, int64_t n_tokens, int n_units, float *dw_b, float *db_b, int accumulate,
```

Result: no change. 90.12 (median of 6 runs) (+0.1%).
